# ultralytics/yolov5

Hardware: NVIDIA H100
Metric: images/sec @640 (forward + NMS) (higher is better)
Workload: dtype bf16

## Files before the change

include/y5b200.h:

```cpp
#ifndef Y5B200_H
#define Y5B200_H
#include <stdint.h>

#if defined(__GNUC__)
#define Y5_API __attribute__((visibility("default")))
#else
#define Y5_API
#endif

#ifdef __cplusplus
extern "C" {
#endif

#define Y5_F16 0
#define Y5_BF16 1
#define Y5_F32 2
#define Y5_U8 3

#define Y5_E_INVALID (-1)
#define Y5_E_UNSUPPORTED (-2)
#define Y5_E_DRIVER (-3)

#define Y5_ACT_NONE 0
#define Y5_ACT_SILU 1
#define Y5_ACT_LEAKY 2

int y5_version(void);
const char* y5_last_error(void);
int64_t y5_launch_count(void);

typedef struct y5_conv_desc {
    const void* in;
    int32_t in_pitch;
    int32_t batch, in_h, in_w, in_c;
    const void* weight;
    const float* bias;
    void* out;
    int32_t out_pitch;
    int32_t out_c;
    const void* residual;
    int32_t res_pitch;
    int32_t ksize, stride, pad;
    int32_t act;
    int32_t dtype;
    int32_t block_k;
    int32_t block_n;
    int32_t kw;
    int32_t pad_w;
    int64_t in_x_stride;
    int64_t in_y_stride;
    int64_t in_n_stride;
    int32_t a_mode;
    int32_t reserved;
    float act_slope;
} y5_conv_desc;

int y5_conv_pick(int32_t in_c, int32_t out_c, int64_t m_rows, int32_t* block_k, int32_t* block_n);

typedef struct y5_conv_plan y5_conv_plan;
int y5_conv_plan_create(const y5_conv_desc* desc, y5_conv_plan** plan);
int y5_conv_plan_run(const y5_conv_plan* plan, void* stream);
void y5_conv_plan_destroy(y5_conv_plan* plan);
struct y5_conv_plan_info {
    int32_t a_mode;
    int32_t tw, th;
    int32_t block_k, block_n, mt;
    int32_t cluster;
    int32_t patch_pw;
    int32_t b_grouped;
    int32_t staged;
    int32_t opt;
    int32_t epi;
    int32_t a_stages, b_stages;
    int32_t grid;
    int32_t tma_epi;
};
int y5_conv_plan_info(const y5_conv_plan* plan, struct y5_conv_plan_info* info);
int y5_conv_bn_silu_fwd(const y5_conv_desc* desc, void* stream);
int y5_conv_direct_fwd(const y5_conv_desc* desc, void* stream);

typedef struct y5_detect_desc {
    const void* in;
    int32_t in_pitch;
    int32_t batch, ny, nx, in_c;
    const void* weight;
    const float* bias;
    void* raw;
    void* z;
    int32_t z_rows, z_row0;
    int32_t na, no, nc;
    float stride;
    float anchor_wh[8];
    int32_t dtype;
    int32_t block_k;
} y5_detect_desc;
typedef struct y5_detect_plan y5_detect_plan;
int y5_detect_plan_create(const y5_detect_desc* desc, y5_detect_plan** plan);
int y5_detect_plan_run(const y5_detect_plan* plan, void* stream);
int y5_detect_plan_run_to(const y5_detect_plan* plan, void* raw, void* z, void* stream);
void y5_detect_plan_destroy(y5_detect_plan* plan);

int y5_stem_s2d(const void* img, int32_t img_dtype, void* out, int32_t out_dtype, int32_t batch, int32_t h, int32_t w,
                int32_t out_row_px, int32_t out_x_off, void* stream);
int y5_sppf_pool(const void* x, int32_t x_pitch, void* y1, void* y2, void* y3, int32_t y_pitch, int32_t batch, int32_t h,
                 int32_t w, int32_t c, int32_t ksize, int32_t dtype, void* stream);
int y5_upsample2x(const void* x, int32_t x_pitch, void* y, int32_t y_pitch, int32_t batch, int32_t h, int32_t w, int32_t c,
                  int32_t dtype, void* stream);
int y5_copy_view(const void* x, int32_t x_pitch, void* y, int32_t y_pitch, int64_t pixels, int32_t c, int32_t dtype,
                 void* stream);
int y5_nhwc_to_nchw(const void* x, int32_t x_pitch, void* y, int32_t batch, int32_t h, int32_t w, int32_t c, int32_t dtype,
                    void* stream);

typedef struct y5_nms_params {
    int32_t batch, n_rows, no, nc, nm;
    int32_t dtype;
    float conf_thres, iou_thres;
    int32_t multi_label, agnostic;
    int32_t max_det;
    int32_t max_nms;
    float max_wh;
    const int32_t* classes;
    int32_t n_classes;
} y5_nms_params;
int64_t y5_nms_workspace_bytes(const y5_nms_params* p);
int y5_nms_batched(const y5_nms_params* p, const void* pred, float* out_rows, int64_t* out_idx, int32_t* out_count,
                   void* workspace, int64_t workspace_bytes, void* stream);
int y5_box_iou(const float* a, int32_t n, const float* b, int32_t m, float eps, float* out, void* stream);

typedef struct y5_loss_params {
    int32_t nl, batch, na, no, nc;
    int32_t ny[5], nx[5];
    int32_t dtype;
    int32_t nt;
    float anchor_t, box_gain, obj_gain, cls_gain, cls_pw, obj_pw, cp, cn;
    float balance[5];
    float grad_scale;
} y5_loss_params;
int64_t y5_loss_workspace_bytes(const y5_loss_params* p);
int y5_loss_fwd_bwd(const y5_loss_params* p, const void* const* pl, const float* targets, const float* anchors,
                    float* out_loss, void* const* grad, void* workspace, int64_t workspace_bytes, void* stream);
int y5_loss_fwd_bwd_scaled(const y5_loss_params* p, const void* const* pl, const float* targets, const float* anchors,
                           float* out_loss, void* const* grad, const float* grad_scale_dev, void* workspace,
                           int64_t workspace_bytes, void* stream);
int y5_loss_read_targets(const y5_loss_params* p, const void* workspace, int32_t level, int64_t* idx5_host,
                         float* tbox_host, int32_t* count_host, void* stream);

int64_t y5_seg_loss_workspace_bytes(const y5_loss_params* p);
int y5_seg_loss_fwd_bwd_scaled(const y5_loss_params* p, const void* const* pl, const float* targets, const float* anchors,
                               const void* proto, int32_t proto_dtype, int64_t ps_b, int64_t ps_k, int64_t ps_y, int64_t ps_x,
                               int32_t nm, int32_t mh, int32_t mw, const float* masks, int32_t n_masks, int32_t gt_h,
                               int32_t gt_w, int32_t overlap, float* out_loss, void* const* grad, void* grad_proto,
                               const float* grad_scale_dev, void* workspace, int64_t workspace_bytes, void* stream);
int y5_seg_loss_read_targets(const y5_loss_params* p, const void* workspace, int32_t level, int64_t* tidx_host,
                             float* xywhn_host, int32_t* count_host, void* stream);

typedef struct y5_wgrad_desc {
    const void* in;
    int32_t in_pitch;
    int32_t batch, in_h, in_w, in_c;
    const void* dout;
    int32_t dout_pitch;
    int32_t out_c;
    float* dweight;
    int32_t ksize, stride, pad;
    int32_t dtype;
    int32_t accumulate;
    int32_t reserved;
    int32_t kw, pad_w;
    int64_t in_x_stride, in_y_stride, in_n_stride;
} y5_wgrad_desc;
int y5_conv_wgrad(const y5_wgrad_desc* d, void* stream);

int64_t y5_bn_workspace_bytes(int32_t channels);
int y5_bn_stats(const void* y, int32_t pitch, int64_t rows, int32_t channels, int32_t dtype, void* workspace,
                void* stream);
int y5_bn_act_fwd(const void* y, int32_t y_pitch, void* z, int32_t z_pitch, int64_t rows, int32_t channels,
                  int32_t dtype, float* mean, float* invstd, const float* gamma, const float* beta, int32_t act,
                  const void* sums, float eps, float momentum, float* running_mean, float* running_var,
                  const void* residual, int32_t res_pitch, void* stream);
int y5_bn_act_bwd(const void* y, int32_t y_pitch, const void* dz, int32_t dz_pitch, void* dy, int32_t dy_pitch,
                  int64_t rows, int32_t channels, int32_t dtype, const float* mean, const float* invstd,
                  const float* gamma, const float* beta, int32_t act, float* dgamma, float* dbeta, void* workspace,
                  void* stream);
int y5_bn_stats_sync(const void* y, int32_t pitch, int64_t rows, int32_t channels, int32_t dtype, void* workspace,
                     void* stream);
int y5_bn_act_fwd_sync(const void* y, int32_t y_pitch, void* z, int32_t z_pitch, int64_t rows, int32_t channels,
                       int32_t dtype, float* mean, float* invstd, const float* gamma, const float* beta, int32_t act,
                       const void* sums, float eps, float momentum, float* running_mean, float* running_var,
                       const void* residual, int32_t res_pitch, void* stream);
int y5_bn_act_bwd_reduce(const void* y, int32_t y_pitch, const void* dz, int32_t dz_pitch, void* dy, int32_t dy_pitch,
                         int64_t rows, int32_t channels, int32_t dtype, const float* mean, const float* invstd,
                         const float* gamma, const float* beta, int32_t act, float* dgamma, float* dbeta, void* workspace,
                         void* stream);
int y5_bn_act_bwd_apply(const void* y, int32_t y_pitch, const void* dz, int32_t dz_pitch, void* dy, int32_t dy_pitch,
                        int64_t rows, int32_t channels, int32_t dtype, const float* mean, const float* invstd,
                        const float* gamma, int32_t act, const void* sums, const void* count, void* stream);
int y5_bn_act_fwd_ex(const void* y, int32_t y_pitch, void* z, int32_t z_pitch, int64_t rows, int32_t channels, int32_t dtype,
                     float* mean, float* invstd, const float* gamma, const float* beta, int32_t act, float slope, const void* sums, float eps,
                     float momentum, float* running_mean, float* running_var, const void* residual, int32_t res_pitch, void* stream);
int y5_bn_act_bwd_ex(const void* y, int32_t y_pitch, const void* dz, int32_t dz_pitch, void* dy, int32_t dy_pitch, int64_t rows,
                     int32_t channels, int32_t dtype, const float* mean, const float* invstd, const float* gamma, const float* beta,
                     int32_t act, float slope, float* dgamma, float* dbeta, void* workspace, void* stream);
int y5_bn_act_fwd_sync_ex(const void* y, int32_t y_pitch, void* z, int32_t z_pitch, int64_t rows, int32_t channels, int32_t dtype,
                          float* mean, float* invstd, const float* gamma, const float* beta, int32_t act, float slope, const void* sums, float eps,
                          float momentum, float* running_mean, float* running_var, const void* residual, int32_t res_pitch, void* stream);
int y5_bn_act_bwd_reduce_ex(const void* y, int32_t y_pitch, const void* dz, int32_t dz_pitch, void* dy, int32_t dy_pitch,
                            int64_t rows, int32_t channels, int32_t dtype, const float* mean, const float* invstd,
                            const float* gamma, const float* beta, int32_t act, float slope, float* dgamma, float* dbeta, void* workspace, void* stream);
int y5_col_sum(const void* y, int32_t pitch, int64_t rows, int32_t channels, int32_t dtype, float* out, void* workspace,
               void* stream);
int y5_weight_pack(const void* w, int32_t w_dtype, int32_t out_c, int32_t in_c, int32_t ksize, void* fwd, int32_t in_c_pad,
                   void* dgrad, int32_t out_c_pad, int32_t dtype, void* stream);
typedef struct y5_pack_item {
    const void* w;
    void* fwd;
    void* dgrad;
    int32_t w_dtype;
    int32_t out_c, in_c, ksize;
    int32_t in_c_pad, out_c_pad;
} y5_pack_item;
int32_t y5_weight_pack_chunk_elems(void);
int y5_weight_pack_multi(const y5_pack_item* items, const int32_t* chunk_item, const int32_t* chunk_index, int32_t n_chunks,
                         int32_t dtype, void* stream);
int y5_upsample2x_bwd(const void* dy, int32_t dy_pitch, void* dx, int32_t dx_pitch, int32_t batch, int32_t h, int32_t w,
                      int32_t c, int32_t dtype, void* stream);
int64_t y5_sppf_bwd_workspace_bytes(int32_t batch, int32_t h, int32_t w, int32_t c);
int y5_sppf_pool_bwd(const void* cat, int32_t cat_pitch, const void* dcat, int32_t dcat_pitch, void* da, int32_t da_pitch,
                     int32_t batch, int32_t h, int32_t w, int32_t c, int32_t ksize, int32_t dtype, void* workspace,
                     void* stream);
int y5_zero_stuff2x(const void* x, int32_t x_pitch, void* y, int32_t y_pitch, int32_t batch, int32_t h, int32_t w,
                    int32_t c, int32_t dtype, void* stream);

typedef struct y5_letterbox_image {
    const void* data;
    int32_t src_h, src_w;
    int32_t row_bytes;
    int32_t new_h, new_w;
    int32_t top, left;
} y5_letterbox_image;
int y5_letterbox_max_images(void);
int y5_letterbox(const y5_letterbox_image* images, int32_t n_images, int32_t out_h, int32_t out_w, int32_t swap_rb,
                 int32_t pad_value, void* out, int32_t out_dtype, int32_t s2d, int32_t out_row_px, int32_t out_x_off,
                 void* stream);

#define Y5_VAL_COPY 0
#define Y5_VAL_LINEAR 1
#define Y5_VAL_AREA 2
struct y5_val_image {
    const void* data;
    void* scratch;
    int32_t src_h, src_w;
    int32_t row_bytes;
    int32_t res_h, res_w;
    int32_t interp;
    int32_t new_h, new_w;
    int32_t top, left;
};
typedef struct y5_val_image y5_val_image;
int y5_val_letterbox(const y5_val_image* images, int32_t n_images, int32_t out_h, int32_t out_w, void* out, int32_t out_dtype,
                     void* stream);

struct y5_cls_image {
    const void* data;
    int32_t side;
    int32_t row_bytes;
};
typedef struct y5_cls_image y5_cls_image;
int y5_cls_batch(const y5_cls_image* images, int32_t n_images, int32_t out_h, int32_t out_w, const float* mean, const float* std, void* out,
                 int32_t out_dtype, void* stream);

int64_t y5_process_mask_workspace_bytes(int32_t n, int32_t mh, int32_t mw, int32_t mode);
int y5_process_mask(const void* protos, int32_t proto_dtype, int32_t batch, int32_t c, int32_t mh, int32_t mw, const float* coef,
                    int32_t coef_stride, const float* boxes, int32_t box_stride, const int32_t* img_index, int32_t n,
                    int32_t in_h, int32_t in_w, int32_t mode, const int32_t* window, void* out, int32_t out_dtype,
                    void* workspace, int64_t workspace_bytes, void* stream);
int y5_crop_mask(const float* masks, const float* boxes, int32_t box_stride, int32_t n, int32_t h, int32_t w, float* out,
                 void* stream);

int y5_scale_boxes(float* boxes, int32_t row_stride, int64_t n_rows, const int32_t* img_index, int32_t rows_per_image,
                   const int32_t* count, const float* meta, void* stream);
int y5_labels_native(const float* targets, int32_t nt, const float* meta, float* out, void* stream);
int y5_match_batch(const float* det, int64_t img_stride, int32_t row_stride, const int32_t* count, int32_t batch,
                   int32_t max_det, const float* labels, int32_t nt, const float* iouv, int32_t niou, float eps,
                   uint8_t* correct, void* stream);
int y5_confusion_batch(const float* det, int64_t img_stride, int32_t row_stride, const int32_t* count, int32_t batch,
                       int32_t max_det, const float* labels, int32_t nt, int32_t nc, float conf_thres, float iou_thres, float eps,
                       int64_t* matrix, int32_t* error, void* stream);

int32_t y5_mask_row_words(int32_t h, int32_t w);
int y5_mask_pack(const void* src, int32_t src_dtype, int32_t src_h, int32_t src_w, int32_t overlap, const float* target_img,
                 int32_t target_stride, int32_t batch, int32_t n_rows, int32_t out_h, int32_t out_w, int32_t* label_index,
                 uint32_t* bits, int32_t* popcount, int32_t* nonbinary, void* stream);
int y5_mask_iou(const uint32_t* gt_bits, const int32_t* gt_pop, const int32_t* label_index, int32_t n_gt, const uint32_t* pred_bits,
                const int32_t* pred_pop, const int32_t* count, int32_t img0, int32_t n_img, int32_t rows_per_image, int32_t words,
                float eps, float* iou, void* stream);
int y5_mask_match_batch(const float* det, int64_t img_stride, int32_t row_stride, const int32_t* count, int32_t batch, int32_t max_det,
                        const float* label_cls, int32_t cls_stride, const int32_t* label_index, int32_t nt, const float* iou,
                        const float* iouv, int32_t niou, uint8_t* correct, void* stream);

typedef struct y5_opt_tensor {
    void* param;
    void* grad;
    void* mom;
    void* ema;
    int64_t numel;
    int32_t group;
    int32_t reserved;
} y5_opt_tensor;
#define Y5_OPT_INV_SCALE 0
#define Y5_OPT_MAX_NORM 1
#define Y5_OPT_EMA_DECAY 2
#define Y5_OPT_EMA_TAU 3
#define Y5_OPT_EMA_UPDATES 4
#define Y5_OPT_OUT_NORM 5
#define Y5_OPT_OUT_SKIPPED 6
#define Y5_OPT_GROUPS 8
int32_t y5_opt_chunk_elems(void);
int y5_opt_step(const y5_opt_tensor* table, const int32_t* chunk_tensor, const int32_t* chunk_index, int32_t n_chunks,
                float* hyper, float* partial, int32_t do_step, int32_t do_ema, int32_t zero_grad, void* stream);

#define Y5_ADAM_LR 0
#define Y5_ADAM_BETA1 1
#define Y5_ADAM_BETA2 2
#define Y5_ADAM_EPS 3
#define Y5_ADAM_WEIGHT_DECAY 4
#define Y5_ADAM_DECOUPLED 5
#define Y5_ADAM_STRIDE 8
int y5_adam_step(const y5_opt_tensor* table, int32_t n_tensors, const int32_t* chunk_tensor, const int32_t* chunk_index, int32_t n_chunks,
                 float* hyper, const double* group_hyper, int64_t sq_offset, float* steps, float* partial, int32_t do_ema,
                 int32_t zero_grad, void* stream);

int y5_grad_pack(const y5_opt_tensor* table, const int32_t* chunk_tensor, const int32_t* chunk_index, int32_t n_chunks,
                 const int64_t* arena_offset, float* arena, float* present, void* stream);
int y5_grad_bind(y5_opt_tensor* arena_table, int32_t n_tensors, const int64_t* arena_offset, float* arena, const float* present,
                 void* stream);

int y5_fold_pack(const void* w, int32_t w_dtype, int32_t out_c, int32_t in_c, int32_t kh, int32_t kw, const void* conv_bias,
                 const void* gamma, const void* beta, const void* mean, const void* var, int32_t bn_dtype, float eps,
                 void* packed, int32_t in_c_pad, int32_t out_c_pad, float* bias_out, int32_t dtype, void* stream);

struct y5_aug_tile {
    const void* src;
    int32_t row_bytes, pixel_stride, channel_stride;
    int32_t x1a, y1a, x2a, y2a;
    int32_t dx, dy;
    int32_t reserved;
};
typedef struct y5_aug_tile y5_aug_tile;
struct y5_aug_image {
    double inv_m[2][6];
    double m[2][6];
    double mix_r;
    float scale[2];
    float clip_max;
    int32_t n_mosaic;
    int32_t n_tiles[2];
    int32_t canvas_w, canvas_h;
    int32_t warp[2];
    int32_t hsv, flipud, fliplr;
    int32_t reserved;
    y5_aug_tile tiles[8];
    uint8_t lut[3][256];
};
typedef struct y5_aug_image y5_aug_image;
#define Y5_AUG_CLIP 1
#define Y5_AUG_IN_XYXY 2
#define Y5_AUG_OUT_XYXY 4
struct y5_aug_label {
    float cls, x, y, w, h;
    float tile_w, tile_h, pad_w, pad_h;
    int32_t image, mosaic, flags;
};
typedef struct y5_aug_label y5_aug_label;
int y5_aug_gather(const y5_aug_image* table, int32_t n_images, int32_t out_h, int32_t out_w, int32_t hsv_simd_cols, int32_t swap_rb,
                  void* out, int32_t out_dtype, int32_t s2d, int32_t out_row_px, int32_t out_x_off, void* stream);
int y5_aug_labels(const y5_aug_image* table, int32_t n_images, const y5_aug_label* labels, int32_t n_labels, int32_t out_h,
                  int32_t out_w, float* targets, int32_t* count, void* stream);

#define Y5_SEG_POINTS 1000
#define Y5_SEG_I32 4
struct y5_aug_segment {
    int32_t point_offset, n_points;
};
typedef struct y5_aug_segment y5_aug_segment;
int y5_seg_warp(const y5_aug_image* table, int32_t n_images, const y5_aug_label* labels, const y5_aug_segment* segments,
                const float* points, int32_t max_points, int32_t n_labels, int32_t out_h, int32_t out_w, int32_t* verts, float* rows,
                int32_t* keep, void* stream);
int y5_seg_raster(const int32_t* verts, int32_t n_verts, const int32_t* keep, int32_t n_labels, int32_t out_h, int32_t out_w,
                  int32_t ratio, uint8_t* masks, int32_t* areas, void* stream);
int y5_seg_order(const int32_t* image_rows, int32_t n_images, const int32_t* keep, const int32_t* areas, const float* rows,
                 int32_t overlap, float* targets, int32_t* plane, int32_t* counts, void* stream);
int y5_seg_compose(const y5_aug_image* table, const y5_aug_label* labels, const int32_t* counts, const int32_t* plane,
                   const uint8_t* masks, int32_t n_out, int32_t mask_h, int32_t mask_w, int32_t overlap, void* out, int32_t out_dtype,
                   void* stream);

int y5_global_avg_pool(const void* x, int32_t x_pitch, void* y, int32_t y_pitch, int32_t batch, int32_t h, int32_t w, int32_t c,
                       int32_t dtype, void* stream);
int y5_global_avg_pool_bwd(const void* dy, int32_t dy_pitch, void* dx, int32_t dx_pitch, int32_t batch, int32_t h, int32_t w, int32_t c,
                           int32_t dtype, void* stream);
int y5_cross_entropy(const void* logits, int32_t dtype, int32_t batch, int32_t nc, int64_t row_stride, const int64_t* labels,
                     float label_smoothing, const float* grad_scale, void* dlogits, int64_t dlogits_stride, float* row_loss, float* loss,
                     void* stream);

#define Y5_AP_META 5
int64_t y5_ap_workspace_bytes(int32_t n_img, int32_t rows_per_image, int32_t niou, int32_t nt, int32_t sets);
int y5_ap_per_class(const uint8_t* tp, const uint8_t* tp2, int64_t tp_img_stride, int32_t tp_row_stride, const float* conf,
                    const float* pred_cls, int64_t img_stride, int32_t row_stride, const int32_t* count, int32_t n_img,
                    int32_t rows_per_image, int32_t niou, const float* target_cls, int32_t nt, const double* grid, double eps,
                    void* workspace, int64_t workspace_bytes, double* out, int32_t* meta, void* stream);

#ifdef __cplusplus
}
#endif
#endif
```

yolov5_b200/_lib.py:

```python
from __future__ import annotations

import ctypes as C
import os

import torch

_HERE = os.path.dirname(os.path.abspath(__file__))
LIB_PATH = os.environ.get("Y5B200_LIB") or os.path.join(_HERE, "liby5b200.so")

Y5_F16, Y5_BF16, Y5_F32, Y5_U8 = 0, 1, 2, 3
ACT_NONE, ACT_SILU, ACT_LEAKY = 0, 1, 2

_DTYPE = {torch.float16: Y5_F16, torch.bfloat16: Y5_BF16, torch.float32: Y5_F32, torch.uint8: Y5_U8}


def dtype_code(dt: torch.dtype) -> int:
    try:
        return _DTYPE[dt]
    except KeyError:
        raise TypeError(f"y5b200: unsupported dtype {dt}") from None


class ConvDesc(C.Structure):
    _fields_ = [
        ("inp", C.c_void_p), ("in_pitch", C.c_int32),
        ("batch", C.c_int32), ("in_h", C.c_int32), ("in_w", C.c_int32), ("in_c", C.c_int32),
        ("weight", C.c_void_p), ("bias", C.c_void_p),
        ("out", C.c_void_p), ("out_pitch", C.c_int32), ("out_c", C.c_int32),
        ("residual", C.c_void_p), ("res_pitch", C.c_int32),
        ("ksize", C.c_int32), ("stride", C.c_int32), ("pad", C.c_int32),
        ("act", C.c_int32), ("dtype", C.c_int32), ("block_k", C.c_int32), ("block_n", C.c_int32),
        ("kw", C.c_int32), ("pad_w", C.c_int32),
        ("in_x_stride", C.c_int64), ("in_y_stride", C.c_int64), ("in_n_stride", C.c_int64),
        ("a_mode", C.c_int32), ("reserved", C.c_int32), ("act_slope", C.c_float),
    ]


class DetectDesc(C.Structure):
    _fields_ = [
        ("inp", C.c_void_p), ("in_pitch", C.c_int32),
        ("batch", C.c_int32), ("ny", C.c_int32), ("nx", C.c_int32), ("in_c", C.c_int32),
        ("weight", C.c_void_p), ("bias", C.c_void_p),
        ("raw", C.c_void_p), ("z", C.c_void_p),
        ("z_rows", C.c_int32), ("z_row0", C.c_int32),
        ("na", C.c_int32), ("no", C.c_int32), ("nc", C.c_int32),
        ("stride", C.c_float), ("anchor_wh", C.c_float * 8),
        ("dtype", C.c_int32), ("block_k", C.c_int32),
    ]


class PlanInfo(C.Structure):
    _fields_ = [
        ("a_mode", C.c_int32), ("tw", C.c_int32), ("th", C.c_int32),
        ("block_k", C.c_int32), ("block_n", C.c_int32), ("mt", C.c_int32), ("cluster", C.c_int32),
        ("patch_pw", C.c_int32), ("b_grouped", C.c_int32), ("staged", C.c_int32), ("opt", C.c_int32), ("epi", C.c_int32),
        ("a_stages", C.c_int32), ("b_stages", C.c_int32), ("grid", C.c_int32),
        ("tma_epi", C.c_int32),
    ]

    def as_dict(self) -> dict:
        return {f: getattr(self, f) for f, _ in self._fields_}


class NmsParams(C.Structure):
    _fields_ = [
        ("batch", C.c_int32), ("n_rows", C.c_int32), ("no", C.c_int32), ("nc", C.c_int32), ("nm", C.c_int32),
        ("dtype", C.c_int32), ("conf_thres", C.c_float), ("iou_thres", C.c_float),
        ("multi_label", C.c_int32), ("agnostic", C.c_int32), ("max_det", C.c_int32), ("max_nms", C.c_int32),
        ("max_wh", C.c_float), ("classes", C.c_void_p), ("n_classes", C.c_int32),
    ]


class LossParams(C.Structure):
    _fields_ = [
        ("nl", C.c_int32), ("batch", C.c_int32), ("na", C.c_int32), ("no", C.c_int32), ("nc", C.c_int32),
        ("ny", C.c_int32 * 5), ("nx", C.c_int32 * 5),
        ("dtype", C.c_int32), ("nt", C.c_int32),
        ("anchor_t", C.c_float), ("box_gain", C.c_float), ("obj_gain", C.c_float), ("cls_gain", C.c_float),
        ("cls_pw", C.c_float), ("obj_pw", C.c_float), ("cp", C.c_float), ("cn", C.c_float),
        ("balance", C.c_float * 5), ("grad_scale", C.c_float),
    ]


class WgradDesc(C.Structure):
    _fields_ = [
        ("inp", C.c_void_p), ("in_pitch", C.c_int32),
        ("batch", C.c_int32), ("in_h", C.c_int32), ("in_w", C.c_int32), ("in_c", C.c_int32),
        ("dout", C.c_void_p), ("dout_pitch", C.c_int32), ("out_c", C.c_int32),
        ("dweight", C.c_void_p),
        ("ksize", C.c_int32), ("stride", C.c_int32), ("pad", C.c_int32),
        ("dtype", C.c_int32), ("accumulate", C.c_int32), ("reserved", C.c_int32),
        ("kw", C.c_int32), ("pad_w", C.c_int32),
        ("in_x_stride", C.c_int64), ("in_y_stride", C.c_int64), ("in_n_stride", C.c_int64),
    ]


class LetterboxImage(C.Structure):
    _fields_ = [
        ("data", C.c_void_p), ("src_h", C.c_int32), ("src_w", C.c_int32), ("row_bytes", C.c_int32),
        ("new_h", C.c_int32), ("new_w", C.c_int32), ("top", C.c_int32), ("left", C.c_int32),
    ]


class ValImage(C.Structure):
    _fields_ = [
        ("data", C.c_void_p), ("scratch", C.c_void_p), ("src_h", C.c_int32), ("src_w", C.c_int32), ("row_bytes", C.c_int32),
        ("res_h", C.c_int32), ("res_w", C.c_int32), ("interp", C.c_int32), ("new_h", C.c_int32), ("new_w", C.c_int32),
        ("top", C.c_int32), ("left", C.c_int32),
    ]


VAL_COPY, VAL_LINEAR, VAL_AREA = 0, 1, 2


class ClsImage(C.Structure):
    _fields_ = [("data", C.c_void_p), ("side", C.c_int32), ("row_bytes", C.c_int32)]


class OptTensor(C.Structure):
    _fields_ = [
        ("param", C.c_void_p), ("grad", C.c_void_p), ("mom", C.c_void_p), ("ema", C.c_void_p),
        ("numel", C.c_int64), ("group", C.c_int32), ("reserved", C.c_int32),
    ]


class PackItem(C.Structure):
    _fields_ = [
        ("w", C.c_void_p), ("fwd", C.c_void_p), ("dgrad", C.c_void_p), ("w_dtype", C.c_int32),
        ("out_c", C.c_int32), ("in_c", C.c_int32), ("ksize", C.c_int32), ("in_c_pad", C.c_int32), ("out_c_pad", C.c_int32),
    ]


class AugTile(C.Structure):
    _fields_ = [
        ("src", C.c_void_p), ("row_bytes", C.c_int32), ("pixel_stride", C.c_int32), ("channel_stride", C.c_int32),
        ("x1a", C.c_int32), ("y1a", C.c_int32), ("x2a", C.c_int32), ("y2a", C.c_int32), ("dx", C.c_int32), ("dy", C.c_int32),
        ("reserved", C.c_int32),
    ]


class AugImage(C.Structure):
    _fields_ = [
        ("inv_m", (C.c_double * 6) * 2), ("m", (C.c_double * 6) * 2), ("mix_r", C.c_double), ("scale", C.c_float * 2),
        ("clip_max", C.c_float), ("n_mosaic", C.c_int32), ("n_tiles", C.c_int32 * 2), ("canvas_w", C.c_int32), ("canvas_h", C.c_int32),
        ("warp", C.c_int32 * 2), ("hsv", C.c_int32), ("flipud", C.c_int32), ("fliplr", C.c_int32), ("reserved", C.c_int32),
        ("tiles", AugTile * 8), ("lut", (C.c_uint8 * 256) * 3),
    ]


class AugLabel(C.Structure):
    _fields_ = [
        ("cls", C.c_float), ("x", C.c_float), ("y", C.c_float), ("w", C.c_float), ("h", C.c_float),
        ("tile_w", C.c_float), ("tile_h", C.c_float), ("pad_w", C.c_float), ("pad_h", C.c_float),
        ("image", C.c_int32), ("mosaic", C.c_int32), ("flags", C.c_int32),
    ]


AUG_CLIP, AUG_IN_XYXY, AUG_OUT_XYXY = 1, 2, 4


class AugSegment(C.Structure):
    _fields_ = [("point_offset", C.c_int32), ("n_points", C.c_int32)]


SEG_POINTS, SEG_I32 = 1000, 4

OPT_INV_SCALE, OPT_MAX_NORM, OPT_EMA_DECAY, OPT_EMA_TAU, OPT_EMA_UPDATES, OPT_OUT_NORM, OPT_OUT_SKIPPED, OPT_GROUPS = 0, 1, 2, 3, 4, 5, 6, 8
ADAM_LR, ADAM_BETA1, ADAM_BETA2, ADAM_EPS, ADAM_WEIGHT_DECAY, ADAM_DECOUPLED, ADAM_STRIDE = 0, 1, 2, 3, 4, 5, 8

_P = C.c_void_p
_I32, _I64, _F = C.c_int32, C.c_int64, C.c_float
SIGNATURES = {
    "y5_version": (_I32, []),
    "y5_last_error": (C.c_char_p, []),
    "y5_launch_count": (_I64, []),
    "y5_conv_pick": (_I32, [_I32, _I32, _I64, C.POINTER(_I32), C.POINTER(_I32)]),
    "y5_conv_plan_create": (_I32, [C.POINTER(ConvDesc), C.POINTER(_P)]),
    "y5_conv_plan_run": (_I32, [_P, _P]),
    "y5_conv_plan_destroy": (None, [_P]),
    "y5_conv_plan_info": (_I32, [_P, C.POINTER(PlanInfo)]),
    "y5_conv_bn_silu_fwd": (_I32, [C.POINTER(ConvDesc), _P]),
    "y5_conv_direct_fwd": (_I32, [C.POINTER(ConvDesc), _P]),
    "y5_detect_plan_create": (_I32, [C.POINTER(DetectDesc), C.POINTER(_P)]),
    "y5_detect_plan_run": (_I32, [_P, _P]),
    "y5_detect_plan_run_to": (_I32, [_P, _P, _P, _P]),
    "y5_detect_plan_destroy": (None, [_P]),
    "y5_stem_s2d": (_I32, [_P, _I32, _P, _I32, _I32, _I32, _I32, _I32, _I32, _P]),
    "y5_sppf_pool": (_I32, [_P, _I32, _P, _P, _P, _I32, _I32, _I32, _I32, _I32, _I32, _I32, _P]),
    "y5_upsample2x": (_I32, [_P, _I32, _P, _I32, _I32, _I32, _I32, _I32, _I32, _P]),
    "y5_copy_view": (_I32, [_P, _I32, _P, _I32, _I64, _I32, _I32, _P]),
    "y5_nhwc_to_nchw": (_I32, [_P, _I32, _P, _I32, _I32, _I32, _I32, _I32, _P]),
    "y5_nms_workspace_bytes": (_I64, [C.POINTER(NmsParams)]),
    "y5_nms_batched": (_I32, [C.POINTER(NmsParams), _P, _P, _P, _P, _P, _I64, _P]),
    "y5_box_iou": (_I32, [_P, _I32, _P, _I32, _F, _P, _P]),
    "y5_loss_workspace_bytes": (_I64, [C.POINTER(LossParams)]),
    "y5_loss_fwd_bwd": (_I32, [C.POINTER(LossParams), C.POINTER(_P), _P, _P, _P, C.POINTER(_P), _P, _I64, _P]),
    "y5_loss_read_targets": (_I32, [C.POINTER(LossParams), _P, _I32, _P, _P, _P, _P]),
    "y5_seg_loss_workspace_bytes": (_I64, [C.POINTER(LossParams)]),
    "y5_seg_loss_fwd_bwd_scaled": (_I32, [C.POINTER(LossParams), C.POINTER(_P), _P, _P, _P, _I32, _I64, _I64, _I64, _I64, _I32, _I32, _I32,
                                          _P, _I32, _I32, _I32, _I32, _P, C.POINTER(_P), _P, _P, _P, _I64, _P]),
    "y5_seg_loss_read_targets": (_I32, [C.POINTER(LossParams), _P, _I32, _P, _P, _P, _P]),
    "y5_conv_wgrad": (_I32, [C.POINTER(WgradDesc), _P]),
    "y5_bn_workspace_bytes": (_I64, [_I32]),
    "y5_bn_stats": (_I32, [_P, _I32, _I64, _I32, _I32, _P, _P]),
    "y5_bn_act_fwd": (_I32, [_P, _I32, _P, _I32, _I64, _I32, _I32, _P, _P, _P, _P, _I32, _P, _F, _F, _P, _P, _P, _I32, _P]),
    "y5_upsample2x_bwd": (_I32, [_P, _I32, _P, _I32, _I32, _I32, _I32, _I32, _I32, _P]),
    "y5_sppf_bwd_workspace_bytes": (_I64, [_I32, _I32, _I32, _I32]),
    "y5_sppf_pool_bwd": (_I32, [_P, _I32, _P, _I32, _P, _I32, _I32, _I32, _I32, _I32, _I32, _I32, _P, _P]),
    "y5_bn_act_bwd": (_I32, [_P, _I32, _P, _I32, _P, _I32, _I64, _I32, _I32, _P, _P, _P, _P, _I32, _P, _P, _P, _P]),
    "y5_col_sum": (_I32, [_P, _I32, _I64, _I32, _I32, _P, _P, _P]),
    "y5_bn_stats_sync": (_I32, [_P, _I32, _I64, _I32, _I32, _P, _P]),
    "y5_bn_act_fwd_sync": (_I32, [_P, _I32, _P, _I32, _I64, _I32, _I32, _P, _P, _P, _P, _I32, _P, _F, _F, _P, _P, _P, _I32, _P]),
    "y5_bn_act_bwd_reduce": (_I32, [_P, _I32, _P, _I32, _P, _I32, _I64, _I32, _I32, _P, _P, _P, _P, _I32, _P, _P, _P, _P]),
    "y5_bn_act_bwd_apply": (_I32, [_P, _I32, _P, _I32, _P, _I32, _I64, _I32, _I32, _P, _P, _P, _I32, _P, _P, _P]),
    "y5_bn_act_fwd_ex": (_I32, [_P, _I32, _P, _I32, _I64, _I32, _I32, _P, _P, _P, _P, _I32, _F, _P, _F, _F, _P, _P, _P, _I32, _P]),
    "y5_bn_act_bwd_ex": (_I32, [_P, _I32, _P, _I32, _P, _I32, _I64, _I32, _I32, _P, _P, _P, _P, _I32, _F, _P, _P, _P, _P]),
    "y5_bn_act_fwd_sync_ex": (_I32, [_P, _I32, _P, _I32, _I64, _I32, _I32, _P, _P, _P, _P, _I32, _F, _P, _F, _F, _P, _P, _P, _I32, _P]),
    "y5_bn_act_bwd_reduce_ex": (_I32, [_P, _I32, _P, _I32, _P, _I32, _I64, _I32, _I32, _P, _P, _P, _P, _I32, _F, _P, _P, _P, _P]),
    "y5_weight_pack": (_I32, [_P, _I32, _I32, _I32, _I32, _P, _I32, _P, _I32, _I32, _P]),
    "y5_weight_pack_chunk_elems": (_I32, []),
    "y5_weight_pack_multi": (_I32, [_P, _P, _P, _I32, _I32, _P]),
    "y5_zero_stuff2x": (_I32, [_P, _I32, _P, _I32, _I32, _I32, _I32, _I32, _I32, _P]),
    "y5_loss_fwd_bwd_scaled": (_I32, [C.POINTER(LossParams), C.POINTER(_P), _P, _P, _P, C.POINTER(_P), _P, _P, _I64, _P]),
    "y5_letterbox_max_images": (_I32, []),
    "y5_letterbox": (_I32, [C.POINTER(LetterboxImage), _I32, _I32, _I32, _I32, _I32, _P, _I32, _I32, _I32, _I32, _P]),
    "y5_val_letterbox": (_I32, [C.POINTER(ValImage), _I32, _I32, _I32, _P, _I32, _P]),
    "y5_cls_batch": (_I32, [_P, _I32, _I32, _I32, C.POINTER(_F), C.POINTER(_F), _P, _I32, _P]),
    "y5_process_mask_workspace_bytes": (_I64, [_I32, _I32, _I32, _I32]),
    "y5_process_mask": (_I32, [_P, _I32, _I32, _I32, _I32, _I32, _P, _I32, _P, _I32, _P, _I32, _I32, _I32, _I32, C.POINTER(_I32), _P, _I32, _P, _I64,
                                _P]),
    "y5_crop_mask": (_I32, [_P, _P, _I32, _I32, _I32, _I32, _P, _P]),
    "y5_scale_boxes": (_I32, [_P, _I32, _I64, _P, _I32, _P, _P, _P]),
    "y5_labels_native": (_I32, [_P, _I32, _P, _P, _P]),
    "y5_match_batch": (_I32, [_P, _I64, _I32, _P, _I32, _I32, _P, _I32, _P, _I32, _F, _P, _P]),
    "y5_confusion_batch": (_I32, [_P, _I64, _I32, _P, _I32, _I32, _P, _I32, _I32, _F, _F, _F, _P, _P, _P]),
    "y5_mask_row_words": (_I32, [_I32, _I32]),
    "y5_mask_pack": (_I32, [_P, _I32, _I32, _I32, _I32, _P, _I32, _I32, _I32, _I32, _I32, _P, _P, _P, _P, _P]),
    "y5_mask_iou": (_I32, [_P, _P, _P, _I32, _P, _P, _P, _I32, _I32, _I32, _I32, _F, _P, _P]),
    "y5_mask_match_batch": (_I32, [_P, _I64, _I32, _P, _I32, _I32, _P, _I32, _P, _I32, _P, _P, _I32, _P, _P]),
    "y5_opt_chunk_elems": (_I32, []),
    "y5_opt_step": (_I32, [_P, _P, _P, _I32, _P, _P, _I32, _I32, _I32, _P]),
    "y5_adam_step": (_I32, [_P, _I32, _P, _P, _I32, _P, _P, _I64, _P, _P, _I32, _I32, _P]),
    "y5_grad_pack": (_I32, [_P, _P, _P, _I32, _P, _P, _P, _P]),
    "y5_grad_bind": (_I32, [_P, _I32, _P, _P, _P, _P]),
    "y5_aug_gather": (_I32, [_P, _I32, _I32, _I32, _I32, _I32, _P, _I32, _I32, _I32, _I32, _P]),
    "y5_aug_labels": (_I32, [_P, _I32, _P, _I32, _I32, _I32, _P, _P, _P]),
    "y5_seg_warp": (_I32, [_P, _I32, _P, _P, _P, _I32, _I32, _I32, _I32, _P, _P, _P, _P]),
    "y5_seg_raster": (_I32, [_P, _I32, _P, _I32, _I32, _I32, _I32, _P, _P, _P]),
    "y5_seg_order": (_I32, [_P, _I32, _P, _P, _P, _I32, _P, _P, _P, _P]),
    "y5_seg_compose": (_I32, [_P, _P, _P, _P, _P, _I32, _I32, _I32, _I32, _P, _I32, _P]),
    "y5_fold_pack": (_I32, [_P, _I32, _I32, _I32, _I32, _I32, _P, _P, _P, _P, _P, _I32, _F, _P, _I32, _I32, _P, _I32, _P]),
    "y5_global_avg_pool": (_I32, [_P, _I32, _P, _I32, _I32, _I32, _I32, _I32, _I32, _P]),
    "y5_global_avg_pool_bwd": (_I32, [_P, _I32, _P, _I32, _I32, _I32, _I32, _I32, _I32, _P]),
    "y5_cross_entropy": (_I32, [_P, _I32, _I32, _I32, _I64, _P, _F, _P, _P, _I64, _P, _P, _P]),
    "y5_ap_workspace_bytes": (_I64, [_I32, _I32, _I32, _I32, _I32]),
    "y5_ap_per_class": (_I32, [_P, _P, _I64, _I32, _P, _P, _I64, _I32, _P, _I32, _I32, _I32, _P, _I32, _P, C.c_double, _P, _I64, _P, _P, _P]),
}

AP_META = 5

_lib = None


def lib():
    global _lib
    if _lib is None:
        if not os.path.exists(LIB_PATH):
            raise RuntimeError(
                f"y5b200: {LIB_PATH} not found -- build it with `python -m yolov5_b200.build` "
                "(or __graft_entry__.build()); this engine has no CPU / PyTorch fallback"
            )
        handle = C.CDLL(LIB_PATH)
        for name, (res, args) in SIGNATURES.items():
            fn = getattr(handle, name)
            fn.restype = res
            fn.argtypes = args
        _lib = handle
    return _lib


def check(code: int, what: str = "") -> None:
    if code != 0:
        msg = lib().y5_last_error().decode(errors="replace")
        raise RuntimeError(f"y5b200 {what} failed (code {code}): {msg}")


def stream_ptr(device=None) -> int:
    return torch.cuda.current_stream(device).cuda_stream


def on(device):
    return torch.cuda.device(device)


def launch_count() -> int:
    return int(lib().y5_launch_count())
```

yolov5_b200/csrc/conv_gemm.cu:

```cuda
#include <cmath>
#include <cstdio>
#include <cstdlib>
#include <cstring>
#include <mutex>
#include <type_traits>

#include "../../include/y5b200.h"
#include "common.cuh"
#include "host_util.h"
#include "wgmma.cuh"

namespace y5 {

constexpr int kBlockM = 128;
constexpr int kConsumers = 2;
constexpr int kConsumerThreads = 128 * kConsumers;
constexpr int kThreads = 128 + kConsumerThreads;
constexpr int kMaxStages = 8;
constexpr int kHeadN = 128;
constexpr int kHeadMaxNo = 8192;
constexpr int kHeadMaxNc = 4096;

__host__ __device__ inline int head_stage_cols(int no) { return no < kHeadN ? no : kHeadN; }

enum AMode { A_LINEAR = 0, A_IM2COL = 1, A_PATCH = 2 };

struct ConvParams {
    int M, N;
    int num_m_tiles;
    int num_m_super, num_n_tiles;
    int kh, kw, c_chunks;
    int block_k;
    int a_mode;
    int Ho, Wo, HoWo, stride, pad_h, pad_w;
    int tw, th, tiles_x, tiles_y;
    int b_grouped;
    int patch_pw;
    int cluster_n;
    uint32_t stg_bytes;
    int tma_epi;
    uint32_t b_sub_bytes;
    float rcp_per_img, rcp_tiles_x, rcp_HoWo, rcp_Wo;
    int a_stages, b_stages;
    uint32_t a_sub_bytes, a_stage_bytes, b_stage_bytes;
    int is_bf16, act;
    const float* bias;
    int bias_n;
    void* out;
    int out_pitch;
    const void* res;
    int res_pitch;
    void* raw;
    void* z;
    int na, no, nc, nx, z_rows, z_row0;
    float det_stride;
    float anchor_wh[8];
    float slope;
};

struct SmemLayout {
    uint32_t off_a, off_b, off_out, off_bias, off_bars, total;
};

__host__ __device__ inline SmemLayout smem_layout(int epi, int no, int bias_n, int a_stages, int b_stages, uint32_t a_bytes,
                                                   uint32_t b_bytes, uint32_t stg_bytes) {
    SmemLayout L;
    uint32_t o = 0;
    L.off_a = o;
    o += a_stages * a_bytes;
    L.off_b = o;
    o += b_stages * b_bytes;
    o = (o + 1023) & ~1023u;
    L.off_out = o;
    if (epi == 1) o += 4 * ((kBlockM * head_stage_cols(no) * 2 + 1023) & ~1023u);
    else o += stg_bytes;
    L.off_bias = o;
    o += ((bias_n + 3) & ~3) * 4;
    o = (o + 7) & ~7u;
    L.off_bars = o;
    o += (4 * kMaxStages + 2) * 8;
    L.total = o;
    return L;
}

__device__ __forceinline__ int fdiv(int n, int d, float rd) {
    if (n >= (1 << 23)) return n / d;
    int q = __float2int_rz(__int2float_rz(n) * rd);
    const int r = n - q * d;
    if (r >= d) ++q;
    else if (r < 0) --q;
    return q;
}

template <int BLOCK_N>
struct EpiBox {
    static constexpr int kRB = BLOCK_N * 2 < 128 ? BLOCK_N * 2 : 128;
    static constexpr int kCols = kRB / 2;
    static constexpr int kNB = BLOCK_N / kCols;
    static constexpr uint32_t kBytes = 64u * kRB;
};
struct EpiOrigin {
    int x, y, img;
};
__device__ __forceinline__ EpiOrigin epi_origin(const ConvParams& p, int mt, int wg) {
    if (p.a_mode != A_PATCH) return {0, mt * kBlockM + 64 * wg, 0};
    const int per_img = p.tiles_x * p.tiles_y;
    const int img = fdiv(mt, per_img, p.rcp_per_img);
    const int rem = mt - img * per_img;
    const int ty = fdiv(rem, p.tiles_x, p.rcp_tiles_x);
    const int x = (rem - ty * p.tiles_x) * p.tw, y = ty * p.th;
    return p.tw > 64 ? EpiOrigin{x + 64 * wg, y, img} : EpiOrigin{x, y + wg * (64 / p.tw), img};
}

template <int BLOCK_N, int MT, int KS, bool BF16>
__device__ __forceinline__ void mma_batch(float (&acc)[MT][BLOCK_N / 2], uint32_t a_lo, uint32_t a_sub16, uint32_t a_hi, uint32_t b_lo,
                                          uint32_t b_hi, uint32_t scale_first) {
    wgmma_fence();
#pragma unroll
    for (int k = 0; k < KS; ++k)
#pragma unroll
        for (int mi = 0; mi < MT; ++mi)
            Wgmma<BLOCK_N>::template run<BF16, 0, 0>(acc[mi], gmma_desc(a_lo + mi * a_sub16 + 2 * k, a_hi), gmma_desc(b_lo + 2 * k, b_hi),
                                                     k == 0 ? scale_first : 1u);
    wgmma_commit();
}

template <int BLOCK_N, int EPI, int MT, bool OPT, bool BF16>
__global__ void __launch_bounds__(kThreads, 1)
conv_gemm_kernel(const __grid_constant__ CUtensorMap tmA, const __grid_constant__ CUtensorMap tmB, const __grid_constant__ CUtensorMap tmO,
                 const __grid_constant__ CUtensorMap tmR, const ConvParams p) {
    static_assert(MT * BLOCK_N <= 256, "accumulators: at most 128 fp32 registers per consumer thread");
    constexpr bool kConv = EPI != 1;
    constexpr bool kLeaky = EPI == 2;
    constexpr int kAcc = BLOCK_N / 2;
    using Box = EpiBox<BLOCK_N>;
    const bool tma_epi = kConv && !OPT && p.tma_epi;

    extern __shared__ __align__(1024) uint8_t smem_raw[];
    uint8_t* smem = reinterpret_cast<uint8_t*>((reinterpret_cast<uintptr_t>(smem_raw) + 1023) & ~uintptr_t(1023));
    const SmemLayout L = smem_layout(EPI, p.no, p.bias_n, p.a_stages, p.b_stages, p.a_stage_bytes, p.b_stage_bytes, p.stg_bytes);
    uint8_t* sA = smem + L.off_a;
    uint8_t* sB = smem + L.off_b;
    float* sBias = reinterpret_cast<float*>(smem + L.off_bias);
    uint64_t* a_full = reinterpret_cast<uint64_t*>(smem + L.off_bars);
    uint64_t* a_empty = a_full + kMaxStages;
    uint64_t* b_full = a_empty + kMaxStages;
    uint64_t* b_empty = b_full + kMaxStages;
    uint64_t* res_full = b_empty + kMaxStages;
    uint64_t* stg_free = res_full + 1;
    uint8_t* stg = smem + L.off_out;

    const int warp = threadIdx.x >> 5;
    const int lane = threadIdx.x & 31;
    const int csize = OPT ? static_cast<int>(cluster_nctarank()) : 1;
    const uint32_t crank = OPT ? cluster_ctarank() : 0u;

    if (threadIdx.x == 0) {
        tma_prefetch_desc(&tmA);
        tma_prefetch_desc(&tmB);
        for (int s = 0; s < kMaxStages; ++s) {
            mbar_init(&a_full[s], 1);
            mbar_init(&a_empty[s], kConsumers);
            mbar_init(&b_full[s], 1);
            mbar_init(&b_empty[s], kConsumers * csize);
        }
        mbar_init(res_full, 1);
        mbar_init(stg_free, kConsumers);
        if (tma_epi) {
            tma_prefetch_desc(&tmO);
            if (p.res) tma_prefetch_desc(&tmR);
        }
        fence_barrier_init();
    }
    if (threadIdx.x >= 128)
        for (int i = threadIdx.x - 128; i < p.bias_n; i += kConsumerThreads) {
            const float b = i < p.N ? __ldg(p.bias + i) : 0.0f;
            sBias[i] = (kConv && p.act) ? 0.5f * b : b;
        }
    __syncthreads();
    if (csize > 1) cluster_sync_all();
    griddep_wait();
    griddep_launch_dependents();

    const int nn = p.num_n_tiles;
    const int num_tiles = ((p.num_m_super + csize - 1) / csize) * nn;
    const int tile0 = blockIdx.x / csize, tile_step = gridDim.x / csize;
    const uint32_t row_bytes = p.block_k * 2;
    const bool patch = p.a_mode == A_PATCH;
    const bool wide = OPT && p.patch_pw > 0;
    const int grp = wide ? p.kh * p.kw : (patch ? p.kh : 1);
    const int num_groups = wide ? p.c_chunks : (patch ? p.c_chunks * p.kw : p.kh * p.kw * p.c_chunks);

    if (warp < 4) {
        setmaxnreg_dec<56>();
    }
    if (warp == 0) {
        int as = 0, bs = 0;
        uint32_t aph = 0, bph = 0, sph = 0;
        for (int tile = tile0; tile < num_tiles; tile += tile_step) {
            const int ms = (tile / nn) * csize + static_cast<int>(crank);
            const int n0 = (tile - (tile / nn) * nn) * BLOCK_N;
            int img[MT], y0[MT], x0[MT];
#pragma unroll
            for (int mi = 0; mi < MT; ++mi) {
                const int mt = ms * MT + mi;
                img[mi] = y0[mi] = x0[mi] = 0;
                if (p.a_mode == A_IM2COL) {
                    const int m0 = mt * kBlockM;
                    img[mi] = fdiv(m0, p.HoWo, p.rcp_HoWo);
                    const int rem = m0 - img[mi] * p.HoWo;
                    const int oy = fdiv(rem, p.Wo, p.rcp_Wo);
                    y0[mi] = oy * p.stride - p.pad_h;
                    x0[mi] = (rem - oy * p.Wo) * p.stride - p.pad_w;
                } else if (patch) {
                    const int per_img = p.tiles_x * p.tiles_y;
                    img[mi] = fdiv(mt, per_img, p.rcp_per_img);
                    const int rem = mt - img[mi] * per_img;
                    const int ty = fdiv(rem, p.tiles_x, p.rcp_tiles_x);
                    y0[mi] = ty * p.th - p.pad_h;
                    x0[mi] = (rem - ty * p.tiles_x) * p.tw - p.pad_w;
                }
            }
            auto issue_group = [&](int cc, int s, int r0) {
                mbar_wait(&a_empty[as], aph ^ 1);
                if (elect_one()) {
                    mbar_arrive_expect_tx(&a_full[as], p.a_stage_bytes);
#pragma unroll
                    for (int mi = 0; mi < MT; ++mi) {
                        uint8_t* a_dst = sA + as * p.a_stage_bytes + mi * p.a_sub_bytes;
                        if (wide) {
                            if (mi == 0) tma_load_4d(&tmA, &a_full[as], a_dst, cc * p.block_k, x0[0], y0[0], img[0]);
                        } else if (p.a_mode == A_LINEAR) tma_load_2d(&tmA, &a_full[as], a_dst, cc * p.block_k, (ms * MT + mi) * kBlockM);
                        else if (p.a_mode == A_IM2COL)
                            tma_load_im2col_4d(&tmA, &a_full[as], a_dst, cc * p.block_k, x0[mi], y0[mi], img[mi], static_cast<uint16_t>(s),
                                               static_cast<uint16_t>(r0));
                        else tma_load_4d(&tmA, &a_full[as], a_dst, cc * p.block_k, x0[mi] + s, y0[mi], img[mi]);
                    }
                }
                __syncwarp();
                if (++as == p.a_stages) { as = 0; aph ^= 1; }
                for (int j = 0; j < grp; ++j) {
                    const int r = patch ? j : r0;
                    const int kb = wide ? j * p.c_chunks + cc : (r * p.kw + s) * p.c_chunks + cc;
                    const bool stage_first = !p.b_grouped || j == 0, stage_last = !p.b_grouped || j == grp - 1;
                    if (stage_first) mbar_wait(&b_empty[bs], bph ^ 1);
                    if (elect_one()) {
                        if (stage_first) mbar_arrive_expect_tx(&b_full[bs], p.b_stage_bytes);
                        uint8_t* b_dst = sB + bs * p.b_stage_bytes + (p.b_grouped ? j * p.b_sub_bytes : 0u);
                        if (csize == 1) tma_load_2d(&tmB, &b_full[bs], b_dst, kb * p.block_k, n0);
                        else {
                            const int slice_rows = BLOCK_N / csize;
                            tma_load_2d_mcast(&tmB, &b_full[bs], b_dst + crank * slice_rows * row_bytes, kb * p.block_k,
                                              n0 + static_cast<int>(crank) * slice_rows, static_cast<uint16_t>((1u << csize) - 1u));
                        }
                    }
                    __syncwarp();
                    if (stage_last && ++bs == p.b_stages) { bs = 0; bph ^= 1; }
                }
            };
            if (wide) {
                for (int cc = 0; cc < p.c_chunks; ++cc) issue_group(cc, 0, 0);
            } else if (patch) {
                for (int cc = 0; cc < p.c_chunks; ++cc)
                    for (int s = 0; s < p.kw; ++s) issue_group(cc, s, 0);
            } else {
                for (int r = 0; r < p.kh; ++r)
                    for (int s = 0; s < p.kw; ++s)
                        for (int cc = 0; cc < p.c_chunks; ++cc) issue_group(cc, s, r);
            }
            if (tma_epi) {
                mbar_wait(stg_free, sph ^ 1);
                if (elect_one()) {
                    if (p.res) {
                        mbar_arrive_expect_tx(res_full, p.stg_bytes);
#pragma unroll 1
                        for (int i = 0; i < kConsumers * MT; ++i) {
                            const EpiOrigin o = epi_origin(p, ms * MT + i % MT, i / MT);
#pragma unroll
                            for (int b = 0; b < Box::kNB; ++b) {
                                uint8_t* dst = stg + (i * Box::kNB + b) * Box::kBytes;
                                if (patch) tma_load_4d(&tmR, res_full, dst, n0 + b * Box::kCols, o.x, o.y, o.img);
                                else tma_load_2d(&tmR, res_full, dst, n0 + b * Box::kCols, o.y);
                            }
                        }
                    } else {
                        mbar_arrive(res_full);
                    }
                }
                __syncwarp();
                sph ^= 1;
            }
        }
    } else if (warp >= 4) {
    setmaxnreg_inc<224>();
    const int wg = (warp >> 2) - 1;
    const int ct = threadIdx.x - 128;
    const int wrow = wg * 64 + (warp & 3) * 16 + (lane >> 2);
    const int ccol = 2 * (lane & 3);
    const bool signal = (threadIdx.x & 127) == 0;
    constexpr bool bf16 = BF16;
    const uint32_t dhi = gmma_desc_hi(row_bytes);
    const uint32_t a_hi = wide ? (dhi & ~0x3FFFu) | (((static_cast<uint32_t>(p.patch_pw) * row_bytes) >> 4) & 0x3FFFu) : dhi;
    const uint32_t a_base = gmma_desc_lo(smem_u32(sA) + (wide ? wg * 8 * p.patch_pw : wg * 64) * row_bytes), b_base = gmma_desc_lo(smem_u32(sB));
    const uint32_t row16 = row_bytes >> 4;
    const uint32_t a_stage16 = p.a_stage_bytes >> 4, b_stage16 = p.b_stage_bytes >> 4, a_sub16 = p.a_sub_bytes >> 4;
    const uint32_t b_sub16 = p.b_sub_bytes >> 4;
    const uint32_t a_shift16 = patch ? (p.tw * row_bytes) >> 4 : 0;
    const int k_steps = p.block_k / 16;
    const int per_img = p.tiles_x * p.tiles_y;
    const int tw_shift = patch ? __ffs(p.tw) - 1 : 0;
    int as = 0, bs = 0, head_set = 0;
    uint32_t aph = 0, bph = 0, rph = 0;
    float acc[MT][kAcc];
#pragma unroll
    for (int mi = 0; mi < MT; ++mi)
#pragma unroll
        for (int i = 0; i < kAcc; ++i) acc[mi][i] = 0.0f;

    int pend_as = 0, pend_bs = 0;
    bool pend_a_last = false, pend_b_last = false;
    auto release_pending = [&]() {
        if (!signal) return;
        if (pend_b_last) {
            if (csize == 1) mbar_arrive(&b_empty[pend_bs]);
            else
                for (int r = 0; r < csize; ++r) mbar_arrive_cluster(mapa_u32(&b_empty[pend_bs], static_cast<uint32_t>(r)));
        }
        if (pend_a_last) mbar_arrive(&a_empty[pend_as]);
    };

    for (int tile = tile0; tile < num_tiles; tile += tile_step) {
        const int ms = (tile / nn) * csize + static_cast<int>(crank);
        const int nt = tile - (tile / nn) * nn;
        const int n0 = nt * BLOCK_N;
        for (int g = 0; g < num_groups; ++g) {
            mbar_wait(&a_full[as], aph);
            const uint32_t a_stage_lo = a_base + as * a_stage16;
            uint32_t a_lo = a_stage_lo;
            for (int j = 0; j < grp; ++j) {
                if (wide) {
                    const int tr = j / p.kw, ts = j - tr * p.kw;
                    a_lo = a_stage_lo + (tr * p.patch_pw + ts) * row16;
                }
                const bool stage_first = !p.b_grouped || j == 0, stage_last = !p.b_grouped || j == grp - 1;
                if (stage_first) mbar_wait(&b_full[bs], bph);
                const uint32_t b_lo = b_base + bs * b_stage16 + (p.b_grouped ? j * b_sub16 : 0u);
                const uint32_t scale_first = (g | j) != 0 ? 1u : 0u;
#pragma unroll
                for (int mi = 0; mi < MT; ++mi) fence_regs(acc[mi]);
                switch (k_steps) {
                    case 4: mma_batch<BLOCK_N, MT, 4, BF16>(acc, a_lo, a_sub16, a_hi, b_lo, dhi, scale_first); break;
                    case 2: mma_batch<BLOCK_N, MT, 2, BF16>(acc, a_lo, a_sub16, a_hi, b_lo, dhi, scale_first); break;
                    default: mma_batch<BLOCK_N, MT, 1, BF16>(acc, a_lo, a_sub16, a_hi, b_lo, dhi, scale_first); break;
                }
                wgmma_wait<1>();
#pragma unroll
                for (int mi = 0; mi < MT; ++mi) fence_regs(acc[mi]);
                if (g | j) release_pending();
                else if (tma_epi && signal && tile != tile0) {
                    tma_store_wait_read0();
                    mbar_arrive(stg_free);
                }
                pend_as = as;
                pend_a_last = j == grp - 1;
                pend_bs = bs;
                pend_b_last = stage_last;
                if (stage_last && ++bs == p.b_stages) { bs = 0; bph ^= 1; }
                a_lo += a_shift16;
            }
            if (++as == p.a_stages) { as = 0; aph ^= 1; }
        }
        wgmma_wait<0>();
#pragma unroll
        for (int mi = 0; mi < MT; ++mi) fence_regs(acc[mi]);
        release_pending();

        if (kConv) {
            const bool staged = OPT && p.stg_bytes != 0;
            const uint32_t stg_pitch = BLOCK_N * 2 + 16;
            uint8_t* stg_wg = stg + wg * 64 * stg_pitch;
            constexpr int kChunks = Box::kRB / 16;
            uint32_t stg_row = smem_u32(stg) + wg * MT * Box::kNB * Box::kBytes + (wrow - wg * 64) * Box::kRB + ccol * 2;
            uint32_t stg_swz = ((((wrow - wg * 64) * Box::kRB) >> 7) & (kChunks - 1)) << 4;
            asm volatile("" : "+r"(stg_row), "+r"(stg_swz));
            auto stg_word = [&](int mi, int h, int j) -> uint32_t {
                return stg_row + (mi * Box::kNB + j / kChunks) * Box::kBytes + h * 8 * Box::kRB + (((j % kChunks) << 4) ^ stg_swz);
            };
            auto pixel_of = [&](int mt, int row) -> long long {
                if (patch) {
                    const int img = fdiv(mt, per_img, p.rcp_per_img);
                    const int rem = mt - img * per_img;
                    const int tyi = fdiv(rem, p.tiles_x, p.rcp_tiles_x);
                    const int oy = tyi * p.th + (row >> tw_shift), ox = (rem - tyi * p.tiles_x) * p.tw + (row & ((1 << tw_shift) - 1));
                    return (mt < p.num_m_tiles && oy < p.Ho && ox < p.Wo) ? static_cast<long long>(img) * p.HoWo + oy * p.Wo + ox : -1;
                }
                const long long m = static_cast<long long>(mt) * kBlockM + row;
                return m < p.M ? m : -1;
            };
            constexpr float kTail = BF16 ? 8.0f : 4.0f;
            constexpr int kRows = 2 * MT, kWords = (OPT ? 128 : 256) / BLOCK_N;
            constexpr int kBatch = kWords < 1 ? 1 : (kWords < kRows ? kWords : kRows);
            const bool has_res = p.res != nullptr;
            if (tma_epi) {
                mbar_wait(res_full, rph);
                rph ^= 1;
            }
            auto rows = [&](auto tma_path) {
                constexpr bool TMA = decltype(tma_path)::value;
#pragma unroll
                for (int q0 = 0; q0 < kRows; q0 += kBatch) {
                    uint32_t rv[kBatch][BLOCK_N / 8];
                    long long gp[kBatch];
#pragma unroll
                    for (int q = 0; q < kBatch; ++q) gp[q] = TMA ? 0 : pixel_of(ms * MT + (q0 + q) / 2, wrow + 8 * ((q0 + q) & 1));
                    if (has_res && TMA) {
#pragma unroll
                        for (int q = 0; q < kBatch; ++q)
#pragma unroll
                            for (int j = 0; j < BLOCK_N / 8; ++j) rv[q][j] = ld_shared_u32(stg_word((q0 + q) / 2, (q0 + q) & 1, j));
                    } else if (has_res) {
#pragma unroll
                        for (int q = 0; q < kBatch; ++q) {
                            const uint16_t* rp = reinterpret_cast<const uint16_t*>(p.res) + (gp[q] < 0 ? 0 : gp[q] * p.res_pitch) + n0 + ccol;
#pragma unroll
                            for (int j = 0; j < BLOCK_N / 8; ++j)
                                rv[q][j] = (gp[q] >= 0 && n0 + 8 * j < p.N) ? *reinterpret_cast<const uint32_t*>(rp + 8 * j) : 0u;
                        }
                    }
#pragma unroll
                    for (int q = 0; q < kBatch; ++q) {
                        const int mi = (q0 + q) / 2, h = (q0 + q) & 1;
                        const int mt = ms * MT + mi;
                        const int row = wrow + 8 * h;
                        const long long gpix = gp[q];
                        if (gpix >= 0 || staged) {
                            uint16_t* op = reinterpret_cast<uint16_t*>(p.out) + gpix * p.out_pitch + n0 + ccol;
                            uint8_t* sp = stg_wg + (row - wg * 64) * stg_pitch + ccol * 2;
                            float hmin = 0.0f;
                            auto row_half = [&](auto tail_pass) {
                                constexpr bool TAIL = decltype(tail_pass)::value;
#pragma unroll
                                for (int j = 0; j < BLOCK_N / 8; ++j) {
                                    if (n0 + 8 * j >= p.N) continue;
                                    const float2 b = *reinterpret_cast<const float2*>(sBias + n0 + 8 * j + ccol);
                                    const float a0 = acc[mi][4 * j + 2 * h], a1 = acc[mi][4 * j + 2 * h + 1];
                                    float f0, f1;
                                    if (p.act) {
                                        const float h0 = fmaf(a0, 0.5f, b.x), h1 = fmaf(a1, 0.5f, b.y);
                                        f0 = silu_from_half(h0);
                                        f1 = silu_from_half(h1);
                                        if (TAIL) {
                                            if (h0 < -0.5f * kTail) f0 = silu_tail(2.0f * h0);
                                            if (h1 < -0.5f * kTail) f1 = silu_tail(2.0f * h1);
                                        } else {
                                            hmin = fminf(hmin, fminf(h0, h1));
                                        }
                                    } else {
                                        f0 = a0 + b.x;
                                        f1 = a1 + b.y;
                                        if (kLeaky) {
                                            f0 = f0 > 0.0f ? f0 : p.slope * f0;
                                            f1 = f1 > 0.0f ? f1 : p.slope * f1;
                                        }
                                    }
                                    if (has_res && gpix >= 0) {
                                        const float2 t = unpack2(rv[q][j], bf16);
                                        f0 += t.x;
                                        f1 += t.y;
                                    }
                                    if (TMA) st_shared_u32(stg_word(mi, h, j), pack2(f0, f1, bf16));
                                    else if (staged) *reinterpret_cast<uint32_t*>(sp + 16 * j) = pack2(f0, f1, bf16);
                                    else *reinterpret_cast<uint32_t*>(op + 8 * j) = pack2(f0, f1, bf16);
                                }
                            };
                            row_half(std::false_type{});
                            if (p.act && __any_sync(__activemask(), hmin < -0.5f * kTail)) row_half(std::true_type{});
                        }
                        if (staged && h == 1) {
                            named_bar_sync(2 + wg, 128);
                            constexpr int kSeg = BLOCK_N / 8;
                            for (int i = threadIdx.x & 127; i < 64 * kSeg; i += 128) {
                                const int lrow = i / kSeg, c = i - lrow * kSeg;
                                const long long gp = pixel_of(mt, wg * 64 + lrow);
                                if (gp >= 0 && n0 + 8 * c < p.N)
                                    *reinterpret_cast<uint4*>(reinterpret_cast<uint16_t*>(p.out) + gp * p.out_pitch + n0 + 8 * c) =
                                        *reinterpret_cast<const uint4*>(stg_wg + lrow * stg_pitch + c * 16);
                            }
                            named_bar_sync(2 + wg, 128);
                        }
                    }
                }
            };
            if (tma_epi) rows(std::true_type{});
            else rows(std::false_type{});
            if (tma_epi) {
                fence_proxy_async_smem();
                named_bar_sync(2 + wg, 128);
                if (signal) {
#pragma unroll 1
                    for (int mi = 0; mi < MT; ++mi) {
                        const EpiOrigin o = epi_origin(p, ms * MT + mi, wg);
#pragma unroll
                        for (int b = 0; b < Box::kNB; ++b) {
                            const uint8_t* src = stg + ((wg * MT + mi) * Box::kNB + b) * Box::kBytes;
                            if (patch) tma_store_4d(&tmO, src, n0 + b * Box::kCols, o.x, o.y, o.img);
                            else tma_store_2d(&tmO, src, n0 + b * Box::kCols, o.y);
                        }
                    }
                    tma_store_commit();
                    if (tile + tile_step >= num_tiles) tma_store_wait_all();
                }
            }
        } else {
            const int no = p.no;
            const int tpa = (no + kHeadN - 1) / kHeadN;
            const int scols = head_stage_cols(no);
            const uint32_t blk = (kBlockM * scols * 2 + 1023) & ~1023u;
            const int set = head_set;
            head_set ^= 1;
            uint16_t* stage_raw = reinterpret_cast<uint16_t*>(smem + L.off_out + (2 * set) * blk);
            uint16_t* stage_z = reinterpret_cast<uint16_t*>(smem + L.off_out + (2 * set + 1) * blk);
            const int a = tpa == 1 ? nt : nt / tpa;
            const int c0 = (nt - a * tpa) * kHeadN;
            const int ncol = min(kHeadN, no - c0);
            const float aw = p.anchor_wh[a * 2], ah = p.anchor_wh[a * 2 + 1];
            const int m0 = ms * kBlockM;
            const int rows_here = min(kBlockM, p.M - m0);
            auto stage = [&](auto wide_path) {
                constexpr bool WIDE = decltype(wide_path)::value;
                float bcol[BLOCK_N / 8][2];
                if (WIDE) {
#pragma unroll
                    for (int j = 0; j < BLOCK_N / 8; ++j)
#pragma unroll
                        for (int e = 0; e < 2; ++e) {
                            const int o = 8 * j + ccol + e;
                            bcol[j][e] = o < ncol ? __ldg(p.bias + n0 + o) : 0.0f;
                        }
                }
#pragma unroll
                for (int h = 0; h < 2; ++h) {
                    const int row = wrow + 8 * h;
                    const int m = m0 + row;
                    int gx = 0, gy = 0;
                    if (m < p.M && (!WIDE || c0 == 0)) {
                        const int pix = m - fdiv(m, p.HoWo, p.rcp_HoWo) * p.HoWo;
                        gy = fdiv(pix, p.nx, p.rcp_Wo);
                        gx = pix - gy * p.nx;
                    }
                    const float fgx = static_cast<float>(gx) - 0.5f, fgy = static_cast<float>(gy) - 0.5f;
#pragma unroll
                    for (int j = 0; j < BLOCK_N / 8; ++j) {
#pragma unroll
                        for (int e = 0; e < 2; ++e) {
                            const int o = 8 * j + ccol + e;
                            if (o >= (WIDE ? ncol : no)) continue;
                            const int oc = WIDE ? c0 + o : o;
                            const float x = acc[0][4 * j + 2 * h + e] + (WIDE ? bcol[j][e] : sBias[n0 + o]);
                            float d = x;
                            if (oc < 5 + p.nc) {
                                const float sg = sigmoid_f(x);
                                if (oc == 0) d = (sg * 2.0f + fgx) * p.det_stride;
                                else if (oc == 1) d = (sg * 2.0f + fgy) * p.det_stride;
                                else if (oc == 2) { const float u = sg * 2.0f; d = u * u * aw; }
                                else if (oc == 3) { const float u = sg * 2.0f; d = u * u * ah; }
                                else d = sg;
                            }
                            const int si = row * (WIDE ? kHeadN : no) + o;
                            stage_raw[si] = pack1(x, bf16);
                            stage_z[si] = pack1(d, bf16);
                        }
                    }
                }
            };
            if (tpa > 1) stage(std::true_type{});
            else stage(std::false_type{});
            named_bar_sync(1, kConsumerThreads);
            if (tpa > 1) {
#pragma unroll 1
                for (int which = 0; which < 2; ++which) {
                    uint16_t* base = reinterpret_cast<uint16_t*>(which == 0 ? p.raw : p.z);
                    const uint16_t* src = which == 0 ? stage_raw : stage_z;
                    auto copy = [&](auto vec) {
                        constexpr int V = decltype(vec)::value;
                        using T = std::conditional_t<V == 8, uint4, std::conditional_t<V == 2, uint32_t, uint16_t>>;
                        const int segs = ncol / V;
                        for (int r = ct >> 5; r < rows_here; r += kConsumerThreads / 32) {
                            const int m = m0 + r;
                            const int b = fdiv(m, p.HoWo, p.rcp_HoWo), pix = m - b * p.HoWo;
                            const long long grow = which == 0 ? (static_cast<long long>(b) * p.na + a) * p.HoWo + pix
                                                              : static_cast<long long>(b) * p.z_rows + p.z_row0 + static_cast<long long>(a) * p.HoWo + pix;
                            T* d = reinterpret_cast<T*>(base + grow * no + c0);
                            const T* s = reinterpret_cast<const T*>(src + r * kHeadN);
                            for (int c = lane; c < segs; c += 32) d[c] = s[c];
                        }
                    };
                    const uintptr_t ba = reinterpret_cast<uintptr_t>(base);
                    if ((no & 7) == 0 && (ba & 15) == 0) copy(std::integral_constant<int, 8>{});
                    else if ((no & 1) == 0 && (ba & 3) == 0) copy(std::integral_constant<int, 2>{});
                    else copy(std::integral_constant<int, 1>{});
                }
                continue;
            }
            const int b_lo = fdiv(m0, p.HoWo, p.rcp_HoWo), b_hi = fdiv(m0 + rows_here - 1, p.HoWo, p.rcp_HoWo);
            for (int b = b_lo; b <= b_hi; ++b) {
                const int r_lo = max(b * p.HoWo - m0, 0), r_hi = min((b + 1) * p.HoWo - m0, rows_here);
                const int pix_lo = m0 + r_lo - b * p.HoWo;
                const int n_el = (r_hi - r_lo) * no;
#pragma unroll
                for (int which = 0; which < 2; ++which) {
                    const long long dst_el = which == 0
                        ? ((static_cast<long long>(b) * p.na + a) * p.HoWo + pix_lo) * no
                        : (static_cast<long long>(b) * p.z_rows + p.z_row0 + static_cast<long long>(a) * p.HoWo + pix_lo) * no;
                    uint16_t* dst = reinterpret_cast<uint16_t*>(which == 0 ? p.raw : p.z) + dst_el;
                    const uint16_t* src = (which == 0 ? stage_raw : stage_z) + r_lo * no;
                    if ((((reinterpret_cast<uintptr_t>(dst) | reinterpret_cast<uintptr_t>(src)) & 15) == 0) && (n_el & 7) == 0) {
                        const uint4* s4 = reinterpret_cast<const uint4*>(src);
                        uint4* d4 = reinterpret_cast<uint4*>(dst);
                        for (int i = ct; i < n_el / 8; i += kConsumerThreads) d4[i] = s4[i];
                    } else {
                        for (int i = ct; i < n_el; i += kConsumerThreads) dst[i] = src[i];
                    }
                }
            }
        }
    }
    }
    if (csize > 1) cluster_sync_all();
}

__global__ void conv_direct_kernel(const uint16_t* __restrict__ in, long long xs, long long ys, long long ns, int B, int H,
                                   int W, int Cin, const uint16_t* __restrict__ w, int cin_pad, const float* __restrict__ bias,
                                   uint16_t* out, int out_pitch, int Cout, const uint16_t* res, int res_pitch, int kh, int kw,
                                   int stride, int pad_h, int pad_w, int Ho, int Wo, int act, float slope, int bf16) {
    const long long idx = static_cast<long long>(blockIdx.x) * blockDim.x + threadIdx.x;
    const long long total = static_cast<long long>(B) * Ho * Wo * Cout;
    if (idx >= total) return;
    const int n = static_cast<int>(idx % Cout);
    const long long m = idx / Cout;
    const int ox = static_cast<int>(m % Wo);
    const int oy = static_cast<int>((m / Wo) % Ho);
    const int b = static_cast<int>(m / (static_cast<long long>(Wo) * Ho));
    float acc = 0.0f;
    for (int r = 0; r < kh; ++r) {
        const int iy = oy * stride - pad_h + r;
        if (iy < 0 || iy >= H) continue;
        for (int s = 0; s < kw; ++s) {
            const int ix = ox * stride - pad_w + s;
            if (ix < 0 || ix >= W) continue;
            const uint16_t* ip = in + b * ns + iy * ys + ix * xs;
            const uint16_t* wp = w + (static_cast<long long>(n) * kh * kw + r * kw + s) * cin_pad;
            for (int c = 0; c < Cin; ++c) acc += unpack1(ip[c], bf16) * unpack1(wp[c], bf16);
        }
    }
    float x = acc + bias[n];
    if (act == Y5_ACT_SILU) x = x / (1.0f + expf(-x));
    else if (act == Y5_ACT_LEAKY) x = x > 0.0f ? x : slope * x;
    if (res) x += unpack1(res[m * res_pitch + n], bf16);
    out[m * out_pitch + n] = pack1(x, bf16);
}

}

using namespace y5;

namespace {

int pick_block_k(int in_c) {
    return in_c > 16 ? 64 : 16;
}

void pick_tile(int out_c, int64_t m_tiles, int* block_n, int* mt) {
    const int64_t sms = sm_count();
    if (out_c <= 32) { *block_n = 32; *mt = 4; return; }
    if (out_c <= 64) { *block_n = 64; *mt = 2; return; }
    if (out_c <= 128) {
        *block_n = 128;
        *mt = ((m_tiles + 1) / 2) >= sms ? 2 : 1;
        return;
    }
    const int64_t tiles256 = m_tiles * ((out_c + 255) / 256);
    *block_n = (tiles256 >= 2 * sms && (out_c % 256 == 0 || out_c > 384)) ? 256 : 128;
    *mt = 1;
}

int pick_block_n(int out_c, int64_t m_rows) {
    int bn, mt;
    pick_tile(out_c, m_rows > 0 ? (m_rows + kBlockM - 1) / kBlockM : 1, &bn, &mt);
    return bn;
}

template <int BN, int EPI, int MT, bool OPT>
cudaError_t launch_conv(const CUtensorMap& a, const CUtensorMap& b, const CUtensorMap& o, const CUtensorMap& r, const ConvParams& p,
                        int grid, int cluster, uint32_t smem, cudaStream_t st) {
    auto* kernel = p.is_bf16 ? conv_gemm_kernel<BN, EPI, MT, OPT, true> : conv_gemm_kernel<BN, EPI, MT, OPT, false>;
    const cudaError_t attr_err = ensure_dyn_smem(reinterpret_cast<const void*>(kernel), 227 * 1024);
    if (attr_err != cudaSuccess) return attr_err;
    count_launch();
    if (cluster == 1) return launch_pdl(kernel, dim3(grid), dim3(kThreads), smem, st, a, b, o, r, p);
    static const bool pdl = [] { const char* e = getenv("Y5_PDL"); return !(e && e[0] == '0'); }();
    cudaLaunchConfig_t cfg{};
    cfg.gridDim = dim3(grid);
    cfg.blockDim = dim3(kThreads);
    cfg.dynamicSmemBytes = smem;
    cfg.stream = st;
    cudaLaunchAttribute attr[2];
    attr[0].id = cudaLaunchAttributeClusterDimension;
    attr[0].val.clusterDim.x = cluster;
    attr[0].val.clusterDim.y = 1;
    attr[0].val.clusterDim.z = 1;
    attr[1].id = cudaLaunchAttributeProgrammaticStreamSerialization;
    attr[1].val.programmaticStreamSerializationAllowed = 1;
    cfg.attrs = attr;
    cfg.numAttrs = pdl ? 2 : 1;
    return cudaLaunchKernelEx(&cfg, kernel, a, b, o, r, p);
}

struct PlanCommon {
    CUtensorMap tmA, tmB;
    CUtensorMap tmO, tmR;
    ConvParams p;
    int block_n, epi, mt, grid, cluster;
    uint32_t smem_bytes;
};

int finish_plan(PlanCommon& pc, int block_n, int epi, int mt, int cluster = 1) {
    ConvParams& p = pc.p;
    p.cluster_n = cluster;
    p.a_stage_bytes = mt * p.a_sub_bytes;
    if (p.patch_pw > 0) p.a_stage_bytes = static_cast<uint32_t>(p.th + p.kh - 1) * p.patch_pw * p.block_k * 2;
    p.num_m_super = (p.num_m_tiles + mt - 1) / mt;
    p.num_n_tiles = (p.N + block_n - 1) / block_n;
    p.bias_n = (epi == 1 && p.no > kHeadN) ? 0 : p.num_n_tiles * block_n;
    const uint32_t budget = 225 * 1024 - 1024;
    const bool patch = p.a_mode == A_PATCH;
    int a_st = 0, b_st = 0;
    if (!patch) {
        for (int s = kMaxStages; s >= 2; --s)
            if (smem_layout(epi, p.no, p.bias_n, s, s, p.a_stage_bytes, p.b_stage_bytes, p.stg_bytes).total <= budget) { a_st = b_st = s; break; }
    } else {
        const int b_min = p.b_grouped ? 2 : 3, b_max = p.b_grouped ? 4 : kMaxStages;
        for (int a = 3; a >= 2 && !a_st; --a)
            for (int b = b_max; b >= b_min; --b)
                if (smem_layout(epi, p.no, p.bias_n, a, b, p.a_stage_bytes, p.b_stage_bytes, p.stg_bytes).total <= budget) { a_st = a; b_st = b; break; }
    }
    if (a_st < 2 || b_st < 2) return set_error(Y5_E_UNSUPPORTED, "conv tile does not fit shared memory (block_n %d a %u b %u)", block_n,
                                                p.a_stage_bytes, p.b_stage_bytes);
    p.a_stages = a_st;
    p.b_stages = b_st;
    pc.smem_bytes = smem_layout(epi, p.no, p.bias_n, a_st, b_st, p.a_stage_bytes, p.b_stage_bytes, p.stg_bytes).total + 1024;
    pc.block_n = block_n;
    pc.epi = epi;
    pc.mt = mt;
    pc.cluster = cluster;
    const long long tiles = static_cast<long long>((p.num_m_super + cluster - 1) / cluster) * p.num_n_tiles;
    const int max_clusters = sm_count() / cluster;
    pc.grid = static_cast<int>(tiles < max_clusters ? tiles : max_clusters) * cluster;
    return 0;
}

bool plan_staged(const PlanCommon& pc) { return pc.p.stg_bytes > 0 && !pc.p.tma_epi; }
bool plan_opt(const PlanCommon& pc) { return pc.cluster > 1 || pc.p.patch_pw > 0 || plan_staged(pc); }

int run_plan(const PlanCommon& pc, cudaStream_t st) {
    cudaError_t e = cudaErrorInvalidValue;
    const int key = (plan_opt(pc) ? 100000 : 0) + pc.epi * 10000 + pc.block_n * 10 + pc.mt;
    switch (key) {
        case 324: e = launch_conv<32, 0, 4, false>(pc.tmA, pc.tmB, pc.tmO, pc.tmR, pc.p, pc.grid, pc.cluster, pc.smem_bytes, st); break;
        case 642: e = launch_conv<64, 0, 2, false>(pc.tmA, pc.tmB, pc.tmO, pc.tmR, pc.p, pc.grid, pc.cluster, pc.smem_bytes, st); break;
        case 1281: e = launch_conv<128, 0, 1, false>(pc.tmA, pc.tmB, pc.tmO, pc.tmR, pc.p, pc.grid, pc.cluster, pc.smem_bytes, st); break;
        case 1282: e = launch_conv<128, 0, 2, false>(pc.tmA, pc.tmB, pc.tmO, pc.tmR, pc.p, pc.grid, pc.cluster, pc.smem_bytes, st); break;
        case 2561: e = launch_conv<256, 0, 1, false>(pc.tmA, pc.tmB, pc.tmO, pc.tmR, pc.p, pc.grid, pc.cluster, pc.smem_bytes, st); break;
        case 11281: e = launch_conv<kHeadN, 1, 1, false>(pc.tmA, pc.tmB, pc.tmO, pc.tmR, pc.p, pc.grid, pc.cluster, pc.smem_bytes, st); break;
        case 100324: e = launch_conv<32, 0, 4, true>(pc.tmA, pc.tmB, pc.tmO, pc.tmR, pc.p, pc.grid, pc.cluster, pc.smem_bytes, st); break;
        case 100642: e = launch_conv<64, 0, 2, true>(pc.tmA, pc.tmB, pc.tmO, pc.tmR, pc.p, pc.grid, pc.cluster, pc.smem_bytes, st); break;
        case 101281: e = launch_conv<128, 0, 1, true>(pc.tmA, pc.tmB, pc.tmO, pc.tmR, pc.p, pc.grid, pc.cluster, pc.smem_bytes, st); break;
        case 101282: e = launch_conv<128, 0, 2, true>(pc.tmA, pc.tmB, pc.tmO, pc.tmR, pc.p, pc.grid, pc.cluster, pc.smem_bytes, st); break;
        case 102561: e = launch_conv<256, 0, 1, true>(pc.tmA, pc.tmB, pc.tmO, pc.tmR, pc.p, pc.grid, pc.cluster, pc.smem_bytes, st); break;
        case 20324: e = launch_conv<32, 2, 4, false>(pc.tmA, pc.tmB, pc.tmO, pc.tmR, pc.p, pc.grid, pc.cluster, pc.smem_bytes, st); break;
        case 20642: e = launch_conv<64, 2, 2, false>(pc.tmA, pc.tmB, pc.tmO, pc.tmR, pc.p, pc.grid, pc.cluster, pc.smem_bytes, st); break;
        case 21281: e = launch_conv<128, 2, 1, false>(pc.tmA, pc.tmB, pc.tmO, pc.tmR, pc.p, pc.grid, pc.cluster, pc.smem_bytes, st); break;
        case 21282: e = launch_conv<128, 2, 2, false>(pc.tmA, pc.tmB, pc.tmO, pc.tmR, pc.p, pc.grid, pc.cluster, pc.smem_bytes, st); break;
        case 22561: e = launch_conv<256, 2, 1, false>(pc.tmA, pc.tmB, pc.tmO, pc.tmR, pc.p, pc.grid, pc.cluster, pc.smem_bytes, st); break;
        case 120324: e = launch_conv<32, 2, 4, true>(pc.tmA, pc.tmB, pc.tmO, pc.tmR, pc.p, pc.grid, pc.cluster, pc.smem_bytes, st); break;
        case 120642: e = launch_conv<64, 2, 2, true>(pc.tmA, pc.tmB, pc.tmO, pc.tmR, pc.p, pc.grid, pc.cluster, pc.smem_bytes, st); break;
        case 121281: e = launch_conv<128, 2, 1, true>(pc.tmA, pc.tmB, pc.tmO, pc.tmR, pc.p, pc.grid, pc.cluster, pc.smem_bytes, st); break;
        case 121282: e = launch_conv<128, 2, 2, true>(pc.tmA, pc.tmB, pc.tmO, pc.tmR, pc.p, pc.grid, pc.cluster, pc.smem_bytes, st); break;
        case 122561: e = launch_conv<256, 2, 1, true>(pc.tmA, pc.tmB, pc.tmO, pc.tmR, pc.p, pc.grid, pc.cluster, pc.smem_bytes, st); break;
        default: return set_error(Y5_E_UNSUPPORTED, "conv: no kernel for block_n %d mt %d epi %d", pc.block_n, pc.mt, pc.epi);
    }
    if (e != cudaSuccess) return set_error(int(e), "conv_gemm launch failed: %s", cudaGetErrorString(e));
    return 0;
}

bool aligned16(const void* p) { return (reinterpret_cast<uintptr_t>(p) & 15) == 0; }

struct Geo {
    int kh, kw, pad_h, pad_w, Ho, Wo;
    long long xs, ys, ns;
};
Geo geometry(const y5_conv_desc* d) {
    Geo g;
    g.kh = d->ksize;
    g.kw = d->kw ? d->kw : d->ksize;
    g.pad_h = d->pad;
    g.pad_w = d->kw ? d->pad_w : d->pad;
    g.xs = d->in_x_stride ? d->in_x_stride : d->in_pitch;
    g.ys = d->in_y_stride ? d->in_y_stride : static_cast<long long>(d->in_w) * g.xs;
    g.ns = d->in_n_stride ? d->in_n_stride : static_cast<long long>(d->in_h) * g.ys;
    g.Ho = (d->in_h + 2 * g.pad_h - g.kh) / d->stride + 1;
    g.Wo = (d->in_w + 2 * g.pad_w - g.kw) / d->stride + 1;
    return g;
}

int encode_epi_map(CUtensorMap* map, int dtype, const void* base, int pitch, const ConvParams& p, int batch, int bn, const char* what) {
    const int rb = bn * 2 < 128 ? bn * 2 : 128;
    const cuuint64_t px = static_cast<cuuint64_t>(pitch) * 2;
    if (p.a_mode == A_PATCH) {
        cuuint64_t dims[4] = {(cuuint64_t)p.N, (cuuint64_t)p.Wo, (cuuint64_t)p.Ho, (cuuint64_t)batch};
        cuuint64_t str[3] = {px, px * p.Wo, px * p.HoWo};
        cuuint32_t box[4] = {(cuuint32_t)(rb / 2), (cuuint32_t)(p.tw < 64 ? p.tw : 64), (cuuint32_t)(p.tw < 64 ? 64 / p.tw : 1), 1};
        return encode_tiled(map, dtype, base, 4, dims, str, box, swizzle_for_row_bytes(rb), what);
    }
    cuuint64_t dims[2] = {(cuuint64_t)p.N, (cuuint64_t)p.M};
    cuuint64_t str[1] = {px};
    cuuint32_t box[2] = {(cuuint32_t)(rb / 2), 64};
    return encode_tiled(map, dtype, base, 2, dims, str, box, swizzle_for_row_bytes(rb), what);
}

}

struct y5_conv_plan {
    PlanCommon pc;
};
struct y5_detect_plan {
    PlanCommon pc;
};

extern "C" Y5_API int y5_conv_pick(int32_t in_c, int32_t out_c, int64_t m_rows, int32_t* block_k, int32_t* block_n) {
    if (in_c <= 0 || out_c <= 0) return set_error(Y5_E_INVALID, "y5_conv_pick: non-positive channel count");
    if (block_k) *block_k = pick_block_k(in_c);
    if (block_n) *block_n = pick_block_n(out_c, m_rows);
    return 0;
}

static int validate_conv(const y5_conv_desc* d) {
    if (!d || !d->in || !d->weight || !d->bias || !d->out) return set_error(Y5_E_INVALID, "conv: null pointer");
    if (d->dtype != Y5_F16 && d->dtype != Y5_BF16) return set_error(Y5_E_UNSUPPORTED, "conv: dtype must be fp16/bf16");
    if (d->batch <= 0 || d->in_h <= 0 || d->in_w <= 0 || d->in_c <= 0 || d->out_c <= 0)
        return set_error(Y5_E_INVALID, "conv: non-positive dimension");
    const long long xs = d->in_x_stride ? d->in_x_stride : d->in_pitch;
    if (xs <= 0 || xs % 8 || (d->in_y_stride % 8) || (d->in_n_stride % 8) || d->out_pitch < d->out_c || d->out_pitch % 8 || d->out_c % 8)
        return set_error(Y5_E_INVALID, "conv: strides/pitches/out_c must be multiples of 8 elements and cover the view");
    if (!d->in_x_stride && d->in_pitch < d->in_c) return set_error(Y5_E_INVALID, "conv: in_pitch smaller than in_c");
    if (!aligned16(d->in) || !aligned16(d->out) || !aligned16(d->weight) || (d->residual && !aligned16(d->residual)))
        return set_error(Y5_E_INVALID, "conv: pointers must be 16-byte aligned");
    if (d->residual && (d->res_pitch < d->out_c || d->res_pitch % 8)) return set_error(Y5_E_INVALID, "conv: bad residual pitch");
    if (d->act != Y5_ACT_NONE && d->act != Y5_ACT_SILU && d->act != Y5_ACT_LEAKY)
        return set_error(Y5_E_UNSUPPORTED, "conv: activation code %d unsupported", d->act);
    if (d->act == Y5_ACT_LEAKY && !std::isfinite(d->act_slope)) return set_error(Y5_E_INVALID, "conv: LeakyReLU slope must be finite");
    const int kw = d->kw ? d->kw : d->ksize, pw = d->kw ? d->pad_w : d->pad;
    if (d->ksize < 1 || d->ksize > 7 || kw < 1 || kw > 7 || d->stride < 1 || d->stride > 8 || d->pad < 0 || d->pad > d->ksize || pw < 0 ||
        pw > kw)
        return set_error(Y5_E_UNSUPPORTED, "conv: kernel %dx%d stride %d pad %d,%d unsupported", d->ksize, kw, d->stride, d->pad, pw);
    return 0;
}

extern "C" Y5_API int y5_conv_plan_create(const y5_conv_desc* d, y5_conv_plan** out) {
    if (!out) return set_error(Y5_E_INVALID, "conv: null plan out");
    *out = nullptr;
    if (int e = validate_conv(d)) return e;
    const Geo g = geometry(d);
    if (g.Ho <= 0 || g.Wo <= 0) return set_error(Y5_E_INVALID, "conv: empty output");
    const int64_t M64 = static_cast<int64_t>(d->batch) * g.Ho * g.Wo;
    if (M64 > 0x7fffffff - 256) return set_error(Y5_E_UNSUPPORTED, "conv: more than 2^31 output pixels");
    const int bk = d->block_k ? d->block_k : pick_block_k(d->in_c);
    if (bk != 16 && bk != 32 && bk != 64) return set_error(Y5_E_INVALID, "conv: block_k must be 16/32/64");
    const bool plain = g.kh == 1 && g.kw == 1 && d->stride == 1 && g.pad_h == 0 && g.pad_w == 0 && !d->in_x_stride && !d->in_y_stride &&
                       !d->in_n_stride;
    int best_tw = 0;
    double best_eff = 0.0;
    if (d->stride == 1 && !plain) {
        for (int tw = 8; tw <= 128; tw <<= 1) {
            const int th = 128 / tw;
            const double eff = (double)g.Wo * g.Ho / ((double)((g.Wo + tw - 1) / tw * tw) * ((g.Ho + th - 1) / th * th));
            if (eff > best_eff + 1e-9) { best_eff = eff; best_tw = tw; }
        }
    }
    int a_mode_sel;
    if (plain) a_mode_sel = A_LINEAR;
    else if (d->a_mode == 2 && d->stride != 1) return set_error(Y5_E_INVALID, "conv: patch mode needs stride 1");
    else if (d->a_mode == 2 || (d->a_mode == 0 && d->stride == 1 && best_eff >= 0.75)) a_mode_sel = A_PATCH;
    else a_mode_sel = A_IM2COL;

    int bn = d->block_n, mt_sel = 0, cl_sel = 1;
    {
        int bn_auto = 0;
        pick_tile(d->out_c, (M64 + kBlockM - 1) / kBlockM, &bn_auto, &mt_sel);
        if (!bn) bn = bn_auto;
        else {
            mt_sel = bn < 128 ? 128 / bn : ((d->reserved & 2) && bn == 128 ? 2 : 1);
            cl_sel = (d->reserved >> 8) > 1 ? (d->reserved >> 8) : 1;
            if (d->reserved & 4) cl_sel = 2;
            if (cl_sel != 1 && cl_sel != 2 && cl_sel != 4) return set_error(Y5_E_INVALID, "conv: cluster size must be 1, 2 or 4");
        }
    }
    if (bn != 32 && bn != 64 && bn != 128 && bn != 256) return set_error(Y5_E_INVALID, "conv: block_n must be 32/64/128/256");
    auto* plan = new y5_conv_plan();
    PlanCommon& pc = plan->pc;
    std::memset(&pc.p, 0, sizeof(pc.p));
    ConvParams& p = pc.p;
    p.M = static_cast<int>(M64);
    p.N = d->out_c;
    p.kh = g.kh; p.kw = g.kw;
    p.Ho = g.Ho; p.Wo = g.Wo; p.HoWo = g.Ho * g.Wo;
    p.rcp_HoWo = 1.0f / static_cast<float>(p.HoWo);
    p.rcp_Wo = 1.0f / static_cast<float>(p.Wo);
    p.stride = d->stride;
    p.pad_h = g.pad_h; p.pad_w = g.pad_w;
    p.is_bf16 = d->dtype == Y5_BF16;
    p.act = d->act == Y5_ACT_SILU;
    p.slope = d->act_slope;
    p.bias = d->bias;
    p.out = d->out;
    p.out_pitch = d->out_pitch;
    p.res = d->residual;
    p.res_pitch = d->res_pitch;
    p.block_k = bk;
    p.c_chunks = (d->in_c + bk - 1) / bk;
    const int row_bytes = bk * 2;
    p.b_sub_bytes = bn * row_bytes;
    p.b_stage_bytes = p.b_sub_bytes;
    p.a_mode = a_mode_sel;

    const CUtensorMapSwizzle sw = swizzle_for_row_bytes(row_bytes);
    int e = 0;
    if (p.a_mode == A_LINEAR) {
        p.num_m_tiles = (p.M + kBlockM - 1) / kBlockM;
        p.a_sub_bytes = kBlockM * row_bytes;
        cuuint64_t dims[2] = {(cuuint64_t)d->in_c, (cuuint64_t)p.M};
        cuuint64_t str[1] = {(cuuint64_t)d->in_pitch * 2};
        cuuint32_t box[2] = {(cuuint32_t)bk, kBlockM};
        e = encode_tiled(&pc.tmA, d->dtype, d->in, 2, dims, str, box, sw, "A linear");
    } else if (p.a_mode == A_IM2COL) {
        p.num_m_tiles = (p.M + kBlockM - 1) / kBlockM;
        p.a_sub_bytes = kBlockM * row_bytes;
        e = encode_im2col(&pc.tmA, d->dtype, d->in, d->in_c, d->in_w, d->in_h, d->batch, g.xs, g.ys, g.ns, g.kh, g.kw, d->stride, g.pad_h,
                          g.pad_w, bk, kBlockM, sw);
    } else {
        p.tw = best_tw;
        p.th = 128 / best_tw;
        {
            const int tx8 = (g.Wo + 7) / 8, ty16 = (g.Ho + 15) / 16;
            const double eff8 = (double)g.Wo * g.Ho / ((double)tx8 * 8 * ty16 * 16);
            if ((d->reserved & 128) && !(d->reserved & 32) && row_bytes == 128 && g.kw > 1 && (mt_sel == 1 || (mt_sel == 2 && tx8 % 2 == 0)) &&
                eff8 >= best_eff - 1e-9) {
                p.tw = 8;
                p.th = 16;
                p.patch_pw = 8 * mt_sel + 8;
            }
        }
        if (!p.patch_pw && g.kh > 1 && bn <= 128) {
            p.b_grouped = 1;
            p.b_stage_bytes = g.kh * p.b_sub_bytes;
        }
        p.tiles_x = (g.Wo + p.tw - 1) / p.tw;
        p.tiles_y = (g.Ho + p.th - 1) / p.th;
        p.rcp_tiles_x = 1.0f / static_cast<float>(p.tiles_x);
        p.rcp_per_img = 1.0f / static_cast<float>(p.tiles_x * p.tiles_y);
        p.num_m_tiles = d->batch * p.tiles_x * p.tiles_y;
        p.a_sub_bytes = p.patch_pw ? 8 * row_bytes : (p.th + g.kh - 1) * p.tw * row_bytes;
        cuuint64_t dims[4] = {(cuuint64_t)d->in_c, (cuuint64_t)d->in_w, (cuuint64_t)d->in_h, (cuuint64_t)d->batch};
        cuuint64_t str[3] = {(cuuint64_t)g.xs * 2, (cuuint64_t)g.ys * 2, (cuuint64_t)g.ns * 2};
        cuuint32_t box[4] = {(cuuint32_t)bk, (cuuint32_t)(p.patch_pw ? p.patch_pw : p.tw), (cuuint32_t)(p.th + g.kh - 1), 1};
        e = encode_tiled(&pc.tmA, d->dtype, d->in, 4, dims, str, box, sw, "A patch");
    }
    if (e) { delete plan; return e; }
    const uint64_t ktot = static_cast<uint64_t>(p.kh) * p.kw * p.c_chunks * bk;
    {
        cuuint64_t dims[2] = {ktot, (cuuint64_t)d->out_c};
        cuuint64_t str[1] = {ktot * 2};
        cuuint32_t box[2] = {(cuuint32_t)bk, (cuuint32_t)(bn / cl_sel)};
        e = encode_tiled(&pc.tmB, d->dtype, d->weight, 2, dims, str, box, sw, "B");
    }
    if (e) { delete plan; return e; }
    const bool opt_modes = cl_sel > 1 || p.patch_pw > 0 || (d->reserved & 8);
    const bool stages_first = p.a_mode == A_IM2COL && bn == 256;
    if (!(d->reserved & 16) && !opt_modes && !stages_first) {
        p.tma_epi = 1;
        p.stg_bytes = static_cast<uint32_t>(mt_sel * bn * 256);
        e = encode_epi_map(&pc.tmO, d->dtype, d->out, d->out_pitch, p, d->batch, bn, "output");
        if (!e && d->residual) e = encode_epi_map(&pc.tmR, d->dtype, d->residual, d->res_pitch, p, d->batch, bn, "residual");
        if (e) { delete plan; return e; }
    } else if ((d->reserved & 8) && !(d->reserved & 16)) {
        p.stg_bytes = static_cast<uint32_t>(kConsumers * 64 * (bn * 2 + 16));
    }
    const int epi = d->act == Y5_ACT_LEAKY ? 2 : 0;
    int e2 = finish_plan(pc, bn, epi, mt_sel, cl_sel);
    if (e2 && p.stg_bytes) {
        p.stg_bytes = 0;
        p.tma_epi = 0;
        e2 = finish_plan(pc, bn, epi, mt_sel, cl_sel);
    }
    if (e2) { delete plan; return e2; }
    *out = plan;
    return 0;
}

extern "C" Y5_API int y5_conv_plan_run(const y5_conv_plan* plan, void* stream) {
    if (!plan) return set_error(Y5_E_INVALID, "conv: null plan");
    return run_plan(plan->pc, static_cast<cudaStream_t>(stream));
}
extern "C" Y5_API void y5_conv_plan_destroy(y5_conv_plan* plan) { delete plan; }

extern "C" Y5_API int y5_conv_plan_info(const y5_conv_plan* plan, struct y5_conv_plan_info* out) {
    if (!plan || !out) return set_error(Y5_E_INVALID, "conv: null plan/info");
    const PlanCommon& pc = plan->pc;
    const ConvParams& p = pc.p;
    out->a_mode = p.a_mode;
    out->tw = p.tw;
    out->th = p.th;
    out->block_k = p.block_k;
    out->block_n = pc.block_n;
    out->mt = pc.mt;
    out->cluster = pc.cluster;
    out->patch_pw = p.patch_pw;
    out->b_grouped = p.b_grouped;
    out->staged = plan_staged(pc);
    out->tma_epi = p.tma_epi;
    out->opt = plan_opt(pc);
    out->epi = pc.epi;
    out->a_stages = p.a_stages;
    out->b_stages = p.b_stages;
    out->grid = pc.grid;
    return 0;
}

extern "C" Y5_API int y5_conv_bn_silu_fwd(const y5_conv_desc* d, void* stream) {
    y5_conv_plan* plan = nullptr;
    if (int e = y5_conv_plan_create(d, &plan)) return e;
    const int e = y5_conv_plan_run(plan, stream);
    y5_conv_plan_destroy(plan);
    return e;
}

extern "C" Y5_API int y5_conv_direct_fwd(const y5_conv_desc* d, void* stream) {
    if (int e = validate_conv(d)) return e;
    const Geo g = geometry(d);
    const int bk = d->block_k ? d->block_k : pick_block_k(d->in_c);
    const int cin_pad = (d->in_c + bk - 1) / bk * bk;
    const long long total = static_cast<long long>(d->batch) * g.Ho * g.Wo * d->out_c;
    const int threads = 256;
    const long long blocks = (total + threads - 1) / threads;
    conv_direct_kernel<<<static_cast<unsigned>(blocks), threads, 0, static_cast<cudaStream_t>(stream)>>>(
        static_cast<const uint16_t*>(d->in), g.xs, g.ys, g.ns, d->batch, d->in_h, d->in_w, d->in_c, static_cast<const uint16_t*>(d->weight),
        cin_pad, d->bias, static_cast<uint16_t*>(d->out), d->out_pitch, d->out_c, static_cast<const uint16_t*>(d->residual), d->res_pitch,
        g.kh, g.kw, d->stride, g.pad_h, g.pad_w, g.Ho, g.Wo, d->act, d->act_slope, d->dtype == Y5_BF16);
    count_launch();
    cudaError_t e = cudaGetLastError();
    if (e != cudaSuccess) return set_error(int(e), "conv_direct launch failed: %s", cudaGetErrorString(e));
    return 0;
}

extern "C" Y5_API int y5_detect_plan_create(const y5_detect_desc* d, y5_detect_plan** out) {
    if (!out) return set_error(Y5_E_INVALID, "detect: null plan out");
    *out = nullptr;
    if (!d || !d->in || !d->weight || !d->bias || !d->raw || !d->z) return set_error(Y5_E_INVALID, "detect: null pointer");
    if (d->dtype != Y5_F16 && d->dtype != Y5_BF16) return set_error(Y5_E_UNSUPPORTED, "detect: dtype must be fp16/bf16");
    if (d->na < 1 || d->na > 4 || d->no < 6 || d->no > kHeadMaxNo || d->nc < 1 || d->nc > kHeadMaxNc || 5 + d->nc > d->no)
        return set_error(Y5_E_UNSUPPORTED, "detect: na %d no %d nc %d unsupported (no <= %d, nc <= %d, na <= 4)", d->na, d->no, d->nc,
                         kHeadMaxNo, kHeadMaxNc);
    if (d->in_pitch < d->in_c || d->in_pitch % 8 || !aligned16(d->in) || !aligned16(d->weight))
        return set_error(Y5_E_INVALID, "detect: bad input view");
    const int64_t M64 = static_cast<int64_t>(d->batch) * d->ny * d->nx;
    if (M64 <= 0 || M64 > 0x7fffffff - 256) return set_error(Y5_E_INVALID, "detect: bad pixel count");
    const int bk = d->block_k ? d->block_k : pick_block_k(d->in_c);
    auto* plan = new y5_detect_plan();
    PlanCommon& pc = plan->pc;
    std::memset(&pc.p, 0, sizeof(pc.p));
    ConvParams& p = pc.p;
    p.M = static_cast<int>(M64);
    p.N = d->na * kHeadN * ((d->no + kHeadN - 1) / kHeadN);
    p.kh = p.kw = 1;
    p.Ho = d->ny; p.Wo = d->nx; p.HoWo = d->ny * d->nx;
    p.rcp_HoWo = 1.0f / static_cast<float>(p.HoWo);
    p.rcp_Wo = 1.0f / static_cast<float>(p.Wo);
    p.stride = 1;
    p.is_bf16 = d->dtype == Y5_BF16;
    p.bias = d->bias;
    p.raw = d->raw;
    p.z = d->z;
    p.na = d->na; p.no = d->no; p.nc = d->nc; p.nx = d->nx;
    p.z_rows = d->z_rows; p.z_row0 = d->z_row0;
    p.det_stride = d->stride;
    for (int i = 0; i < 8; ++i) p.anchor_wh[i] = d->anchor_wh[i];
    p.a_mode = A_LINEAR;
    p.block_k = bk;
    p.c_chunks = (d->in_c + bk - 1) / bk;
    const int row_bytes = bk * 2;
    p.a_sub_bytes = kBlockM * row_bytes;
    p.b_stage_bytes = kHeadN * row_bytes;
    p.num_m_tiles = (p.M + kBlockM - 1) / kBlockM;
    const CUtensorMapSwizzle sw = swizzle_for_row_bytes(row_bytes);
    cuuint64_t dims[2] = {(cuuint64_t)d->in_c, (cuuint64_t)p.M};
    cuuint64_t str[1] = {(cuuint64_t)d->in_pitch * 2};
    cuuint32_t box[2] = {(cuuint32_t)bk, kBlockM};
    int e = encode_tiled(&pc.tmA, d->dtype, d->in, 2, dims, str, box, sw, "head A");
    if (e) { delete plan; return e; }
    const uint64_t ktot = static_cast<uint64_t>(p.c_chunks) * bk;
    cuuint64_t bdims[2] = {ktot, (cuuint64_t)p.N};
    cuuint64_t bstr[1] = {ktot * 2};
    cuuint32_t bbox[2] = {(cuuint32_t)bk, (cuuint32_t)kHeadN};
    e = encode_tiled(&pc.tmB, d->dtype, d->weight, 2, bdims, bstr, bbox, sw, "head B");
    if (e) { delete plan; return e; }
    if (int e2 = finish_plan(pc, kHeadN, 1, 1)) { delete plan; return e2; }
    *out = plan;
    return 0;
}
extern "C" Y5_API int y5_detect_plan_run(const y5_detect_plan* plan, void* stream) {
    if (!plan) return set_error(Y5_E_INVALID, "detect: null plan");
    return run_plan(plan->pc, static_cast<cudaStream_t>(stream));
}
extern "C" Y5_API int y5_detect_plan_run_to(const y5_detect_plan* plan, void* raw, void* z, void* stream) {
    if (!plan || !raw || !z) return set_error(Y5_E_INVALID, "detect: null plan/output");
    PlanCommon pc = plan->pc;
    pc.p.raw = raw;
    pc.p.z = z;
    return run_plan(pc, static_cast<cudaStream_t>(stream));
}
extern "C" Y5_API void y5_detect_plan_destroy(y5_detect_plan* plan) { delete plan; }
```

Measured before the change: 3170.

## Add ping-pong consumer warpgroup schedule to conv GEMM kernel

Adds a ping-pong mode in which the two consumer warpgroups work on alternating tiles, each covering the full 128-row M tile. An mbarrier token orders their MMA phases so one warpgroup's epilogue overlaps the other's mainloop. Per-warpgroup staging buffers and residual/stage-free barriers are added, and the staging space is doubled. The plan picker now steers default configs toward 128-wide N with MT=1 so ping-pong applies, and falls back to the cooperative plan when that plan gets deeper pipelining. A host-side schedule checker is also exported, at the cost of more smem and more kernel instantiations.

Measured after the change: 3226 (median of 6 runs). 1.8% higher.

```diff
diff --git a/include/y5b200.h b/include/y5b200.h
--- a/include/y5b200.h
+++ b/include/y5b200.h
@@ -74,8 +74,11 @@
     int32_t a_stages, b_stages;
     int32_t grid;
     int32_t tma_epi;
+    int32_t pingpong;
 };
 int y5_conv_plan_info(const y5_conv_plan* plan, struct y5_conv_plan_info* info);
+int64_t y5_conv_pingpong_check(int32_t num_tiles, int32_t grid, int32_t num_groups, int32_t grp, int32_t b_grouped, int32_t a_stages,
+                               int32_t b_stages, int64_t* fills);
 int y5_conv_bn_silu_fwd(const y5_conv_desc* desc, void* stream);
 int y5_conv_direct_fwd(const y5_conv_desc* desc, void* stream);
 
diff --git a/yolov5_b200/_lib.py b/yolov5_b200/_lib.py
--- a/yolov5_b200/_lib.py
+++ b/yolov5_b200/_lib.py
@@ -55,7 +55,7 @@
         ("block_k", C.c_int32), ("block_n", C.c_int32), ("mt", C.c_int32), ("cluster", C.c_int32),
         ("patch_pw", C.c_int32), ("b_grouped", C.c_int32), ("staged", C.c_int32), ("opt", C.c_int32), ("epi", C.c_int32),
         ("a_stages", C.c_int32), ("b_stages", C.c_int32), ("grid", C.c_int32),
-        ("tma_epi", C.c_int32),
+        ("tma_epi", C.c_int32), ("pingpong", C.c_int32),
     ]
 
     def as_dict(self) -> dict:
@@ -179,6 +179,7 @@
     "y5_conv_plan_run": (_I32, [_P, _P]),
     "y5_conv_plan_destroy": (None, [_P]),
     "y5_conv_plan_info": (_I32, [_P, C.POINTER(PlanInfo)]),
+    "y5_conv_pingpong_check": (_I64, [_I32, _I32, _I32, _I32, _I32, _I32, _I32, C.POINTER(_I64)]),
     "y5_conv_bn_silu_fwd": (_I32, [C.POINTER(ConvDesc), _P]),
     "y5_conv_direct_fwd": (_I32, [C.POINTER(ConvDesc), _P]),
     "y5_detect_plan_create": (_I32, [C.POINTER(DetectDesc), C.POINTER(_P)]),
diff --git a/yolov5_b200/csrc/conv_gemm.cu b/yolov5_b200/csrc/conv_gemm.cu
--- a/yolov5_b200/csrc/conv_gemm.cu
+++ b/yolov5_b200/csrc/conv_gemm.cu
@@ -4,6 +4,7 @@
 #include <cstring>
 #include <mutex>
 #include <type_traits>
+#include <vector>
 
 #include "../../include/y5b200.h"
 #include "common.cuh"
@@ -63,7 +64,7 @@
 };
 
 __host__ __device__ inline SmemLayout smem_layout(int epi, int no, int bias_n, int a_stages, int b_stages, uint32_t a_bytes,
-                                                   uint32_t b_bytes, uint32_t stg_bytes) {
+                                                   uint32_t b_bytes, uint32_t stg_bytes, bool pp) {
     SmemLayout L;
     uint32_t o = 0;
     L.off_a = o;
@@ -78,7 +79,7 @@
     o += ((bias_n + 3) & ~3) * 4;
     o = (o + 7) & ~7u;
     L.off_bars = o;
-    o += (4 * kMaxStages + 2) * 8;
+    o += (4 * kMaxStages + (pp ? 6 : 2)) * 8;
     L.total = o;
     return L;
 }
@@ -90,6 +91,19 @@
     if (r >= d) ++q;
     else if (r < 0) --q;
     return q;
+}
+
+struct TileStages {
+    int a, b;
+};
+__host__ __device__ inline TileStages tile_stages(int num_groups, int grp, int b_grouped) {
+    return {num_groups, b_grouped ? num_groups : num_groups * grp};
+}
+__host__ __device__ inline void ring_advance(int& idx, uint32_t& phase, int n, int stages) {
+    idx += n;
+    const int wraps = idx / stages;
+    idx -= wraps * stages;
+    phase ^= static_cast<uint32_t>(wraps & 1);
 }
 
 template <int BLOCK_N>
@@ -112,33 +126,36 @@
     return p.tw > 64 ? EpiOrigin{x + 64 * wg, y, img} : EpiOrigin{x, y + wg * (64 / p.tw), img};
 }
 
-template <int BLOCK_N, int MT, int KS, bool BF16>
-__device__ __forceinline__ void mma_batch(float (&acc)[MT][BLOCK_N / 2], uint32_t a_lo, uint32_t a_sub16, uint32_t a_hi, uint32_t b_lo,
-                                          uint32_t b_hi, uint32_t scale_first) {
+template <int BLOCK_N, int NV, int VP, int KS, bool BF16>
+__device__ __forceinline__ void mma_batch(float (&acc)[NV][BLOCK_N / 2], uint32_t a_lo, uint32_t a_sub16, uint32_t a_half16, uint32_t a_hi,
+                                          uint32_t b_lo, uint32_t b_hi, uint32_t scale_first) {
     wgmma_fence();
 #pragma unroll
     for (int k = 0; k < KS; ++k)
 #pragma unroll
-        for (int mi = 0; mi < MT; ++mi)
-            Wgmma<BLOCK_N>::template run<BF16, 0, 0>(acc[mi], gmma_desc(a_lo + mi * a_sub16 + 2 * k, a_hi), gmma_desc(b_lo + 2 * k, b_hi),
-                                                     k == 0 ? scale_first : 1u);
+        for (int v = 0; v < NV; ++v)
+            Wgmma<BLOCK_N>::template run<BF16, 0, 0>(acc[v], gmma_desc(a_lo + (v / VP) * a_sub16 + (v % VP) * a_half16 + 2 * k, a_hi),
+                                                     gmma_desc(b_lo + 2 * k, b_hi), k == 0 ? scale_first : 1u);
     wgmma_commit();
 }
 
-template <int BLOCK_N, int EPI, int MT, bool OPT, bool BF16>
+template <int BLOCK_N, int EPI, int MT, bool OPT, bool BF16, bool PP>
 __global__ void __launch_bounds__(kThreads, 1)
 conv_gemm_kernel(const __grid_constant__ CUtensorMap tmA, const __grid_constant__ CUtensorMap tmB, const __grid_constant__ CUtensorMap tmO,
                  const __grid_constant__ CUtensorMap tmR, const ConvParams p) {
     static_assert(MT * BLOCK_N <= 256, "accumulators: at most 128 fp32 registers per consumer thread");
+    static_assert(!PP || (MT * BLOCK_N <= 128 && EPI != 1 && !OPT), "ping-pong: conv epilogue, default instantiation, 128 accumulators");
     constexpr bool kConv = EPI != 1;
     constexpr bool kLeaky = EPI == 2;
     constexpr int kAcc = BLOCK_N / 2;
+    constexpr int kVP = PP ? 2 : 1;
+    constexpr int kV = MT * kVP;
     using Box = EpiBox<BLOCK_N>;
-    const bool tma_epi = kConv && !OPT && p.tma_epi;
+    const bool tma_epi = kConv && !OPT && (PP || p.tma_epi);
 
     extern __shared__ __align__(1024) uint8_t smem_raw[];
     uint8_t* smem = reinterpret_cast<uint8_t*>((reinterpret_cast<uintptr_t>(smem_raw) + 1023) & ~uintptr_t(1023));
-    const SmemLayout L = smem_layout(EPI, p.no, p.bias_n, p.a_stages, p.b_stages, p.a_stage_bytes, p.b_stage_bytes, p.stg_bytes);
+    const SmemLayout L = smem_layout(EPI, p.no, p.bias_n, p.a_stages, p.b_stages, p.a_stage_bytes, p.b_stage_bytes, p.stg_bytes, PP);
     uint8_t* sA = smem + L.off_a;
     uint8_t* sB = smem + L.off_b;
     float* sBias = reinterpret_cast<float*>(smem + L.off_bias);
@@ -147,8 +164,10 @@
     uint64_t* b_full = a_empty + kMaxStages;
     uint64_t* b_empty = b_full + kMaxStages;
     uint64_t* res_full = b_empty + kMaxStages;
-    uint64_t* stg_free = res_full + 1;
+    uint64_t* stg_free = res_full + kVP;
+    uint64_t* mma_tok = stg_free + kVP;
     uint8_t* stg = smem + L.off_out;
+    const uint32_t stg_blk = p.stg_bytes / kVP;
 
     const int warp = threadIdx.x >> 5;
     const int lane = threadIdx.x & 31;
@@ -160,12 +179,16 @@
         tma_prefetch_desc(&tmB);
         for (int s = 0; s < kMaxStages; ++s) {
             mbar_init(&a_full[s], 1);
-            mbar_init(&a_empty[s], kConsumers);
+            mbar_init(&a_empty[s], PP ? 1 : kConsumers);
             mbar_init(&b_full[s], 1);
-            mbar_init(&b_empty[s], kConsumers * csize);
-        }
-        mbar_init(res_full, 1);
-        mbar_init(stg_free, kConsumers);
+            mbar_init(&b_empty[s], (PP ? 1 : kConsumers) * csize);
+        }
+        for (int w = 0; w < kVP; ++w) {
+            mbar_init(&res_full[w], 1);
+            mbar_init(&stg_free[w], PP ? 1 : kConsumers);
+        }
+        if (PP)
+            for (int w = 0; w < 2; ++w) mbar_init(&mma_tok[w], 128);
         if (tma_epi) {
             tma_prefetch_desc(&tmO);
             if (p.res) tma_prefetch_desc(&tmR);
@@ -197,7 +220,8 @@
     if (warp == 0) {
         int as = 0, bs = 0;
         uint32_t aph = 0, bph = 0, sph = 0;
-        for (int tile = tile0; tile < num_tiles; tile += tile_step) {
+        int it = 0;
+        for (int tile = tile0; tile < num_tiles; tile += tile_step, ++it) {
             const int ms = (tile / nn) * csize + static_cast<int>(crank);
             const int n0 = (tile - (tile / nn) * nn) * BLOCK_N;
             int img[MT], y0[MT], x0[MT];
@@ -269,40 +293,44 @@
                         for (int cc = 0; cc < p.c_chunks; ++cc) issue_group(cc, s, r);
             }
             if (tma_epi) {
-                mbar_wait(stg_free, sph ^ 1);
+                const int w = PP ? (it & 1) : 0;
+                mbar_wait(&stg_free[w], ((sph >> w) & 1) ^ 1);
                 if (elect_one()) {
                     if (p.res) {
-                        mbar_arrive_expect_tx(res_full, p.stg_bytes);
+                        mbar_arrive_expect_tx(&res_full[w], stg_blk);
 #pragma unroll 1
                         for (int i = 0; i < kConsumers * MT; ++i) {
                             const EpiOrigin o = epi_origin(p, ms * MT + i % MT, i / MT);
 #pragma unroll
                             for (int b = 0; b < Box::kNB; ++b) {
-                                uint8_t* dst = stg + (i * Box::kNB + b) * Box::kBytes;
-                                if (patch) tma_load_4d(&tmR, res_full, dst, n0 + b * Box::kCols, o.x, o.y, o.img);
-                                else tma_load_2d(&tmR, res_full, dst, n0 + b * Box::kCols, o.y);
+                                uint8_t* dst = stg + w * stg_blk + (i * Box::kNB + b) * Box::kBytes;
+                                if (patch) tma_load_4d(&tmR, &res_full[w], dst, n0 + b * Box::kCols, o.x, o.y, o.img);
+                                else tma_load_2d(&tmR, &res_full[w], dst, n0 + b * Box::kCols, o.y);
                             }
                         }
                     } else {
-                        mbar_arrive(res_full);
+                        mbar_arrive(&res_full[w]);
                     }
                 }
                 __syncwarp();
-                sph ^= 1;
+                sph ^= 1u << w;
             }
         }
     } else if (warp >= 4) {
     setmaxnreg_inc<224>();
     const int wg = (warp >> 2) - 1;
     const int ct = threadIdx.x - 128;
-    const int wrow = wg * 64 + (warp & 3) * 16 + (lane >> 2);
+    const int lrow = (warp & 3) * 16 + (lane >> 2);
+    const int wrow = wg * 64 + lrow;
     const int ccol = 2 * (lane & 3);
     const bool signal = (threadIdx.x & 127) == 0;
     constexpr bool bf16 = BF16;
     const uint32_t dhi = gmma_desc_hi(row_bytes);
     const uint32_t a_hi = wide ? (dhi & ~0x3FFFu) | (((static_cast<uint32_t>(p.patch_pw) * row_bytes) >> 4) & 0x3FFFu) : dhi;
-    const uint32_t a_base = gmma_desc_lo(smem_u32(sA) + (wide ? wg * 8 * p.patch_pw : wg * 64) * row_bytes), b_base = gmma_desc_lo(smem_u32(sB));
+    const uint32_t a_base = gmma_desc_lo(smem_u32(sA) + (wide ? wg * 8 * p.patch_pw : (PP ? 0 : wg * 64)) * row_bytes);
+    const uint32_t b_base = gmma_desc_lo(smem_u32(sB));
     const uint32_t row16 = row_bytes >> 4;
+    const uint32_t a_half16 = 64 * row16;
     const uint32_t a_stage16 = p.a_stage_bytes >> 4, b_stage16 = p.b_stage_bytes >> 4, a_sub16 = p.a_sub_bytes >> 4;
     const uint32_t b_sub16 = p.b_sub_bytes >> 4;
     const uint32_t a_shift16 = patch ? (p.tw * row_bytes) >> 4 : 0;
@@ -310,12 +338,18 @@
     const int per_img = p.tiles_x * p.tiles_y;
     const int tw_shift = patch ? __ffs(p.tw) - 1 : 0;
     int as = 0, bs = 0, head_set = 0;
-    uint32_t aph = 0, bph = 0, rph = 0;
-    float acc[MT][kAcc];
-#pragma unroll
-    for (int mi = 0; mi < MT; ++mi)
-#pragma unroll
-        for (int i = 0; i < kAcc; ++i) acc[mi][i] = 0.0f;
+    uint32_t aph = 0, bph = 0, rph = 0, tph = 0;
+    float acc[kV][kAcc];
+#pragma unroll
+    for (int v = 0; v < kV; ++v)
+#pragma unroll
+        for (int i = 0; i < kAcc; ++i) acc[v][i] = 0.0f;
+    const TileStages ts = tile_stages(num_groups, grp, p.b_grouped);
+    const int my_first = PP ? tile0 + wg * tile_step : tile0, my_step = PP ? 2 * tile_step : tile_step;
+    if (PP && wg == 1) {
+        ring_advance(as, aph, ts.a, p.a_stages);
+        ring_advance(bs, bph, ts.b, p.b_stages);
+    }
 
     int pend_as = 0, pend_bs = 0;
     bool pend_a_last = false, pend_b_last = false;
@@ -329,10 +363,15 @@
         if (pend_a_last) mbar_arrive(&a_empty[pend_as]);
     };
 
-    for (int tile = tile0; tile < num_tiles; tile += tile_step) {
+    for (int tile = my_first; tile < num_tiles; tile += my_step) {
         const int ms = (tile / nn) * csize + static_cast<int>(crank);
         const int nt = tile - (tile / nn) * nn;
         const int n0 = nt * BLOCK_N;
+        const bool ordered = PP && tile != tile0;
+        if (ordered) {
+            mbar_wait(&mma_tok[wg], tph);
+            tph ^= 1;
+        }
         for (int g = 0; g < num_groups; ++g) {
             mbar_wait(&a_full[as], aph);
             const uint32_t a_stage_lo = a_base + as * a_stage16;
@@ -347,19 +386,19 @@
                 const uint32_t b_lo = b_base + bs * b_stage16 + (p.b_grouped ? j * b_sub16 : 0u);
                 const uint32_t scale_first = (g | j) != 0 ? 1u : 0u;
 #pragma unroll
-                for (int mi = 0; mi < MT; ++mi) fence_regs(acc[mi]);
+                for (int v = 0; v < kV; ++v) fence_regs(acc[v]);
                 switch (k_steps) {
-                    case 4: mma_batch<BLOCK_N, MT, 4, BF16>(acc, a_lo, a_sub16, a_hi, b_lo, dhi, scale_first); break;
-                    case 2: mma_batch<BLOCK_N, MT, 2, BF16>(acc, a_lo, a_sub16, a_hi, b_lo, dhi, scale_first); break;
-                    default: mma_batch<BLOCK_N, MT, 1, BF16>(acc, a_lo, a_sub16, a_hi, b_lo, dhi, scale_first); break;
+                    case 4: mma_batch<BLOCK_N, kV, kVP, 4, BF16>(acc, a_lo, a_sub16, a_half16, a_hi, b_lo, dhi, scale_first); break;
+                    case 2: mma_batch<BLOCK_N, kV, kVP, 2, BF16>(acc, a_lo, a_sub16, a_half16, a_hi, b_lo, dhi, scale_first); break;
+                    default: mma_batch<BLOCK_N, kV, kVP, 1, BF16>(acc, a_lo, a_sub16, a_half16, a_hi, b_lo, dhi, scale_first); break;
                 }
                 wgmma_wait<1>();
 #pragma unroll
-                for (int mi = 0; mi < MT; ++mi) fence_regs(acc[mi]);
+                for (int v = 0; v < kV; ++v) fence_regs(acc[v]);
                 if (g | j) release_pending();
-                else if (tma_epi && signal && tile != tile0) {
+                else if (tma_epi && signal && tile != my_first) {
                     tma_store_wait_read0();
-                    mbar_arrive(stg_free);
+                    mbar_arrive(&stg_free[PP ? wg : 0]);
                 }
                 pend_as = as;
                 pend_a_last = j == grp - 1;
@@ -370,21 +409,27 @@
             }
             if (++as == p.a_stages) { as = 0; aph ^= 1; }
         }
+        if (PP) mbar_arrive(&mma_tok[wg ^ 1]);
         wgmma_wait<0>();
 #pragma unroll
-        for (int mi = 0; mi < MT; ++mi) fence_regs(acc[mi]);
+        for (int v = 0; v < kV; ++v) fence_regs(acc[v]);
         release_pending();
+        if (PP) {
+            ring_advance(as, aph, ts.a, p.a_stages);
+            ring_advance(bs, bph, ts.b, p.b_stages);
+        }
 
         if (kConv) {
             const bool staged = OPT && p.stg_bytes != 0;
             const uint32_t stg_pitch = BLOCK_N * 2 + 16;
             uint8_t* stg_wg = stg + wg * 64 * stg_pitch;
             constexpr int kChunks = Box::kRB / 16;
-            uint32_t stg_row = smem_u32(stg) + wg * MT * Box::kNB * Box::kBytes + (wrow - wg * 64) * Box::kRB + ccol * 2;
-            uint32_t stg_swz = ((((wrow - wg * 64) * Box::kRB) >> 7) & (kChunks - 1)) << 4;
+            uint32_t stg_row = smem_u32(stg) + wg * kV * Box::kNB * Box::kBytes + lrow * Box::kRB + ccol * 2;
+            uint32_t stg_swz = (((lrow * Box::kRB) >> 7) & (kChunks - 1)) << 4;
             asm volatile("" : "+r"(stg_row), "+r"(stg_swz));
-            auto stg_word = [&](int mi, int h, int j) -> uint32_t {
-                return stg_row + (mi * Box::kNB + j / kChunks) * Box::kBytes + h * 8 * Box::kRB + (((j % kChunks) << 4) ^ stg_swz);
+            auto stg_word = [&](int v, int h, int j) -> uint32_t {
+                const int slot = PP ? (v % kVP) * MT + v / kVP : v;
+                return stg_row + (slot * Box::kNB + j / kChunks) * Box::kBytes + h * 8 * Box::kRB + (((j % kChunks) << 4) ^ stg_swz);
             };
             auto pixel_of = [&](int mt, int row) -> long long {
                 if (patch) {
@@ -398,11 +443,11 @@
                 return m < p.M ? m : -1;
             };
             constexpr float kTail = BF16 ? 8.0f : 4.0f;
-            constexpr int kRows = 2 * MT, kWords = (OPT ? 128 : 256) / BLOCK_N;
+            constexpr int kRows = 2 * kV, kWords = (OPT ? 128 : 256) / BLOCK_N;
             constexpr int kBatch = kWords < 1 ? 1 : (kWords < kRows ? kWords : kRows);
             const bool has_res = p.res != nullptr;
             if (tma_epi) {
-                mbar_wait(res_full, rph);
+                mbar_wait(&res_full[PP ? wg : 0], rph);
                 rph ^= 1;
             }
             auto rows = [&](auto tma_path) {
@@ -429,7 +474,8 @@
                     }
 #pragma unroll
                     for (int q = 0; q < kBatch; ++q) {
-                        const int mi = (q0 + q) / 2, h = (q0 + q) & 1;
+                        const int v = (q0 + q) / 2, h = (q0 + q) & 1;
+                        const int mi = v / kVP;
                         const int mt = ms * MT + mi;
                         const int row = wrow + 8 * h;
                         const long long gpix = gp[q];
@@ -443,7 +489,7 @@
                                 for (int j = 0; j < BLOCK_N / 8; ++j) {
                                     if (n0 + 8 * j >= p.N) continue;
                                     const float2 b = *reinterpret_cast<const float2*>(sBias + n0 + 8 * j + ccol);
-                                    const float a0 = acc[mi][4 * j + 2 * h], a1 = acc[mi][4 * j + 2 * h + 1];
+                                    const float a0 = acc[v][4 * j + 2 * h], a1 = acc[v][4 * j + 2 * h + 1];
                                     float f0, f1;
                                     if (p.act) {
                                         const float h0 = fmaf(a0, 0.5f, b.x), h1 = fmaf(a1, 0.5f, b.y);
@@ -468,7 +514,7 @@
                                         f0 += t.x;
                                         f1 += t.y;
                                     }
-                                    if (TMA) st_shared_u32(stg_word(mi, h, j), pack2(f0, f1, bf16));
+                                    if (TMA) st_shared_u32(stg_word(v, h, j), pack2(f0, f1, bf16));
                                     else if (staged) *reinterpret_cast<uint32_t*>(sp + 16 * j) = pack2(f0, f1, bf16);
                                     else *reinterpret_cast<uint32_t*>(op + 8 * j) = pack2(f0, f1, bf16);
                                 }
@@ -491,24 +537,25 @@
                     }
                 }
             };
-            if (tma_epi) rows(std::true_type{});
+            if constexpr (PP) rows(std::true_type{});
+            else if (tma_epi) rows(std::true_type{});
             else rows(std::false_type{});
             if (tma_epi) {
                 fence_proxy_async_smem();
                 named_bar_sync(2 + wg, 128);
                 if (signal) {
 #pragma unroll 1
-                    for (int mi = 0; mi < MT; ++mi) {
-                        const EpiOrigin o = epi_origin(p, ms * MT + mi, wg);
+                    for (int i = 0; i < kV; ++i) {
+                        const EpiOrigin o = PP ? epi_origin(p, ms * MT + i % MT, i / MT) : epi_origin(p, ms * MT + i, wg);
 #pragma unroll
                         for (int b = 0; b < Box::kNB; ++b) {
-                            const uint8_t* src = stg + ((wg * MT + mi) * Box::kNB + b) * Box::kBytes;
+                            const uint8_t* src = stg + ((wg * kV + i) * Box::kNB + b) * Box::kBytes;
                             if (patch) tma_store_4d(&tmO, src, n0 + b * Box::kCols, o.x, o.y, o.img);
                             else tma_store_2d(&tmO, src, n0 + b * Box::kCols, o.y);
                         }
                     }
                     tma_store_commit();
-                    if (tile + tile_step >= num_tiles) tma_store_wait_all();
+                    if (tile + my_step >= num_tiles) tma_store_wait_all();
                 }
             }
         } else {
@@ -690,10 +737,10 @@
     return bn;
 }
 
-template <int BN, int EPI, int MT, bool OPT>
+template <int BN, int EPI, int MT, bool OPT, bool PP = false>
 cudaError_t launch_conv(const CUtensorMap& a, const CUtensorMap& b, const CUtensorMap& o, const CUtensorMap& r, const ConvParams& p,
                         int grid, int cluster, uint32_t smem, cudaStream_t st) {
-    auto* kernel = p.is_bf16 ? conv_gemm_kernel<BN, EPI, MT, OPT, true> : conv_gemm_kernel<BN, EPI, MT, OPT, false>;
+    auto* kernel = p.is_bf16 ? conv_gemm_kernel<BN, EPI, MT, OPT, true, PP> : conv_gemm_kernel<BN, EPI, MT, OPT, false, PP>;
     const cudaError_t attr_err = ensure_dyn_smem(reinterpret_cast<const void*>(kernel), 227 * 1024);
     if (attr_err != cudaSuccess) return attr_err;
     count_launch();
@@ -721,6 +768,7 @@
     CUtensorMap tmO, tmR;
     ConvParams p;
     int block_n, epi, mt, grid, cluster;
+    int pingpong;
     uint32_t smem_bytes;
 };
 
@@ -737,18 +785,18 @@
     int a_st = 0, b_st = 0;
     if (!patch) {
         for (int s = kMaxStages; s >= 2; --s)
-            if (smem_layout(epi, p.no, p.bias_n, s, s, p.a_stage_bytes, p.b_stage_bytes, p.stg_bytes).total <= budget) { a_st = b_st = s; break; }
+            if (smem_layout(epi, p.no, p.bias_n, s, s, p.a_stage_bytes, p.b_stage_bytes, p.stg_bytes, pc.pingpong).total <= budget) { a_st = b_st = s; break; }
     } else {
         const int b_min = p.b_grouped ? 2 : 3, b_max = p.b_grouped ? 4 : kMaxStages;
         for (int a = 3; a >= 2 && !a_st; --a)
             for (int b = b_max; b >= b_min; --b)
-                if (smem_layout(epi, p.no, p.bias_n, a, b, p.a_stage_bytes, p.b_stage_bytes, p.stg_bytes).total <= budget) { a_st = a; b_st = b; break; }
+                if (smem_layout(epi, p.no, p.bias_n, a, b, p.a_stage_bytes, p.b_stage_bytes, p.stg_bytes, pc.pingpong).total <= budget) { a_st = a; b_st = b; break; }
     }
     if (a_st < 2 || b_st < 2) return set_error(Y5_E_UNSUPPORTED, "conv tile does not fit shared memory (block_n %d a %u b %u)", block_n,
                                                 p.a_stage_bytes, p.b_stage_bytes);
     p.a_stages = a_st;
     p.b_stages = b_st;
-    pc.smem_bytes = smem_layout(epi, p.no, p.bias_n, a_st, b_st, p.a_stage_bytes, p.b_stage_bytes, p.stg_bytes).total + 1024;
+    pc.smem_bytes = smem_layout(epi, p.no, p.bias_n, a_st, b_st, p.a_stage_bytes, p.b_stage_bytes, p.stg_bytes, pc.pingpong).total + 1024;
     pc.block_n = block_n;
     pc.epi = epi;
     pc.mt = mt;
@@ -764,8 +812,14 @@
 
 int run_plan(const PlanCommon& pc, cudaStream_t st) {
     cudaError_t e = cudaErrorInvalidValue;
-    const int key = (plan_opt(pc) ? 100000 : 0) + pc.epi * 10000 + pc.block_n * 10 + pc.mt;
+    const int key = (plan_opt(pc) ? 100000 : 0) + (pc.pingpong ? 200000 : 0) + pc.epi * 10000 + pc.block_n * 10 + pc.mt;
     switch (key) {
+        case 200324: e = launch_conv<32, 0, 4, false, true>(pc.tmA, pc.tmB, pc.tmO, pc.tmR, pc.p, pc.grid, pc.cluster, pc.smem_bytes, st); break;
+        case 200642: e = launch_conv<64, 0, 2, false, true>(pc.tmA, pc.tmB, pc.tmO, pc.tmR, pc.p, pc.grid, pc.cluster, pc.smem_bytes, st); break;
+        case 201281: e = launch_conv<128, 0, 1, false, true>(pc.tmA, pc.tmB, pc.tmO, pc.tmR, pc.p, pc.grid, pc.cluster, pc.smem_bytes, st); break;
+        case 220324: e = launch_conv<32, 2, 4, false, true>(pc.tmA, pc.tmB, pc.tmO, pc.tmR, pc.p, pc.grid, pc.cluster, pc.smem_bytes, st); break;
+        case 220642: e = launch_conv<64, 2, 2, false, true>(pc.tmA, pc.tmB, pc.tmO, pc.tmR, pc.p, pc.grid, pc.cluster, pc.smem_bytes, st); break;
+        case 221281: e = launch_conv<128, 2, 1, false, true>(pc.tmA, pc.tmB, pc.tmO, pc.tmR, pc.p, pc.grid, pc.cluster, pc.smem_bytes, st); break;
         case 324: e = launch_conv<32, 0, 4, false>(pc.tmA, pc.tmB, pc.tmO, pc.tmR, pc.p, pc.grid, pc.cluster, pc.smem_bytes, st); break;
         case 642: e = launch_conv<64, 0, 2, false>(pc.tmA, pc.tmB, pc.tmO, pc.tmR, pc.p, pc.grid, pc.cluster, pc.smem_bytes, st); break;
         case 1281: e = launch_conv<128, 0, 1, false>(pc.tmA, pc.tmB, pc.tmO, pc.tmR, pc.p, pc.grid, pc.cluster, pc.smem_bytes, st); break;
@@ -906,6 +960,11 @@
         }
     }
     if (bn != 32 && bn != 64 && bn != 128 && bn != 256) return set_error(Y5_E_INVALID, "conv: block_n must be 32/64/128/256");
+    const int picked_bn = bn, picked_mt = mt_sel;
+    if (!d->block_n && !(d->reserved & (8 | 16 | 128)) && mt_sel * bn > 128 && !(a_mode_sel == A_IM2COL && bn == 256)) {
+        bn = 128;
+        mt_sel = 1;
+    }
     auto* plan = new y5_conv_plan();
     PlanCommon& pc = plan->pc;
     std::memset(&pc.p, 0, sizeof(pc.p));
@@ -989,6 +1048,8 @@
     if (!(d->reserved & 16) && !opt_modes && !stages_first) {
         p.tma_epi = 1;
         p.stg_bytes = static_cast<uint32_t>(mt_sel * bn * 256);
+        pc.pingpong = mt_sel * bn <= 128 && !(d->reserved & 64);
+        if (pc.pingpong) p.stg_bytes *= 2;
         e = encode_epi_map(&pc.tmO, d->dtype, d->out, d->out_pitch, p, d->batch, bn, "output");
         if (!e && d->residual) e = encode_epi_map(&pc.tmR, d->dtype, d->residual, d->res_pitch, p, d->batch, bn, "residual");
         if (e) { delete plan; return e; }
@@ -997,12 +1058,33 @@
     }
     const int epi = d->act == Y5_ACT_LEAKY ? 2 : 0;
     int e2 = finish_plan(pc, bn, epi, mt_sel, cl_sel);
+    if (e2 && pc.pingpong) {
+        pc.pingpong = 0;
+        p.stg_bytes /= 2;
+        e2 = finish_plan(pc, bn, epi, mt_sel, cl_sel);
+    }
     if (e2 && p.stg_bytes) {
         p.stg_bytes = 0;
         p.tma_epi = 0;
+        pc.pingpong = 0;
         e2 = finish_plan(pc, bn, epi, mt_sel, cl_sel);
     }
     if (e2) { delete plan; return e2; }
+    if (pc.pingpong && !d->block_n) {
+        y5_conv_desc dc = *d;
+        dc.block_n = picked_bn;
+        dc.reserved |= 64 | (picked_bn == 128 && picked_mt == 2 ? 2 : 0);
+        y5_conv_plan* coop = nullptr;
+        if (y5_conv_plan_create(&dc, &coop) == 0) {
+            const ConvParams& q = coop->pc.p;
+            if (q.tma_epi && (q.a_stages > p.a_stages || q.b_stages > p.b_stages)) {
+                delete plan;
+                plan = coop;
+            } else {
+                delete coop;
+            }
+        }
+    }
     *out = plan;
     return 0;
 }
@@ -1028,12 +1110,81 @@
     out->b_grouped = p.b_grouped;
     out->staged = plan_staged(pc);
     out->tma_epi = p.tma_epi;
+    out->pingpong = pc.pingpong;
     out->opt = plan_opt(pc);
     out->epi = pc.epi;
     out->a_stages = p.a_stages;
     out->b_stages = p.b_stages;
     out->grid = pc.grid;
     return 0;
+}
+
+extern "C" Y5_API int64_t y5_conv_pingpong_check(int32_t num_tiles, int32_t grid, int32_t num_groups, int32_t grp, int32_t b_grouped,
+                                                 int32_t a_stages, int32_t b_stages, int64_t* fills) {
+    if (num_tiles < 1 || grid < 1 || num_groups < 1 || grp < 1 || a_stages < 2 || a_stages > kMaxStages || b_stages < 2 ||
+        b_stages > kMaxStages)
+        return set_error(Y5_E_INVALID, "conv_pingpong_check: bad schedule");
+    struct Fill {
+        int idx;
+        uint32_t phase;
+        int owner, releases;
+    };
+    const TileStages ts = tile_stages(num_groups, grp, b_grouped);
+    int64_t bad = 0, nfill = 0;
+    for (int cta = 0; cta < grid; ++cta) {
+        std::vector<Fill> fa, fb;
+        std::vector<size_t> a_first, b_first;
+        int as = 0, bs = 0, it = 0;
+        uint32_t aph = 0, bph = 0;
+        for (int tile = cta; tile < num_tiles; tile += grid, ++it) {
+            a_first.push_back(fa.size());
+            b_first.push_back(fb.size());
+            for (int g = 0; g < num_groups; ++g) {
+                fa.push_back({as, aph, it & 1, 0});
+                if (++as == a_stages) { as = 0; aph ^= 1; }
+                for (int j = 0; j < grp; ++j) {
+                    if (!b_grouped || j == 0) fb.push_back({bs, bph, it & 1, 0});
+                    if ((!b_grouped || j == grp - 1) && ++bs == b_stages) { bs = 0; bph ^= 1; }
+                }
+            }
+        }
+        a_first.push_back(fa.size());
+        b_first.push_back(fb.size());
+        for (int wg = 0; wg < 2; ++wg) {
+            as = bs = 0;
+            aph = bph = 0;
+            if (wg == 1) {
+                ring_advance(as, aph, ts.a, a_stages);
+                ring_advance(bs, bph, ts.b, b_stages);
+            }
+            for (int lt = wg; lt < it; lt += 2) {
+                if (a_first[lt + 1] - a_first[lt] != static_cast<size_t>(ts.a) || b_first[lt + 1] - b_first[lt] != static_cast<size_t>(ts.b)) ++bad;
+                size_t na = a_first[lt], nb = b_first[lt];
+                for (int g = 0; g < num_groups; ++g) {
+                    Fill& fA = fa[na++];
+                    bad += fA.idx != as || fA.phase != aph || fA.owner != wg;
+                    for (int j = 0; j < grp; ++j) {
+                        Fill& fB = fb[nb];
+                        bad += fB.idx != bs || fB.phase != bph || fB.owner != wg;
+                        if (!b_grouped || j == grp - 1) {
+                            ++fB.releases;
+                            ++nb;
+                            if (++bs == b_stages) { bs = 0; bph ^= 1; }
+                        }
+                    }
+                    ++fA.releases;
+                    if (++as == a_stages) { as = 0; aph ^= 1; }
+                }
+                ring_advance(as, aph, ts.a, a_stages);
+                ring_advance(bs, bph, ts.b, b_stages);
+            }
+        }
+        for (const Fill& f : fa) bad += f.releases != 1;
+        for (const Fill& f : fb) bad += f.releases != 1;
+        nfill += static_cast<int64_t>(fa.size() + fb.size());
+    }
+    if (fills) *fills = nfill;
+    return bad;
 }
 
 extern "C" Y5_API int y5_conv_bn_silu_fwd(const y5_conv_desc* d, void* stream) {
```
